# RookieJunChen/FullSubNet-plus

Hardware: AMD Instinct MI355X
Metric: STFT frames/sec (257-bin, 2 s clips), FullSubNet+ forward (higher is better)
Workload: dtype f32

## Files before the change

### fullsubnet_plus_amd/csrc/fsnp_debug_abi.hip

```cpp
#include <algorithm>
#include <string>

#include "fsnp_common.h"
#include "lstm_common.h"
#include "planner.h"
#include "fsnp_handle.h"
#include "weight_layouts.h"
#include "pcm.h"

static double lstm_flops_per_step(const fsnp_handle* h) {
    if (h->sb_tcn) return 8 * (2.0 * h->NIN * h->CH + 2.0 * h->CH * 3 + 2.0 * h->CH * h->NIN) + 2.0 * h->NIN * h->cfg.output_size;
    const double H = h->H, NIN = h->NIN, OUT = h->cfg.output_size, G = h->NG;
    return 2.0 * G * H * (NIN + H) + 2.0 * G * H * (2 * H) + 2.0 * H * OUT;
}
static double tcn_flops_per_frame(const fsnp_handle* h) {
    const double F = h->F, CH = h->CH;
    return h->NB * (2.0 * F * CH + 2.0 * CH * 3 + 2.0 * CH * F) + 2.0 * F * F;
}
static double fb_lstm_flops_per_frame(const fsnp_handle* h) {
    const double F = h->F, CH = h->CH;
    return 2.0 * h->NG * CH * (F + CH) + 2.0 * h->NG * CH * (2 * CH) + 2.0 * CH * F;
}

extern "C" {

int fsnp_read_stage(fsnp_handle* h, const char* name, float* host_out, int64_t numel) {
    if (!h || !name || !host_out) { set_error("fsnp_read_stage: null argument"); return 1; }
    if (!h->have_last) { set_error("fsnp_read_stage: no forward has run"); return 2; }
    const Dims& d = h->last_dims;
    const Workspace& w = h->last_ws;
    const size_t plane = (size_t)d.B * d.Tp * d.FP;
    const std::string n = name;
    const float* src = nullptr;
    bool is_gate = false;
    static const char* tags[3] = {"mag", "real", "imag"};
    for (int b = 0; b < h->NFB; ++b) {
        if (n == std::string("att_") + tags[b]) src = reinterpret_cast<float*>(h->last_base + w.att) + b * plane;
        if (n == std::string("fb_") + tags[b]) src = reinterpret_cast<float*>(h->last_base + w.fb) + b * plane;
        if (h->NFB == 3 && n == std::string("gate_") + tags[b]) { src = reinterpret_cast<float*>(h->last_base + w.gate) + (size_t)b * d.B * d.FP; is_gate = true; }
    }
    if (n == "tcn0_mag") {
        if (!h->debug) { set_error("tcn0_mag needs FSNP_DEBUG_STAGES=1 at fsnp_create time"); return 2; }
        src = reinterpret_cast<float*>(h->last_base + w.dbg_tcn0);
    }
    if (!src) { set_error("unknown stage %s", name); return 2; }
    const int64_t rows = is_gate ? d.B : (int64_t)d.B * d.Tp;
    if (numel != rows * d.F) { set_error("stage %s has %lld elements, caller asked %lld", name, (long long)(rows * d.F), (long long)numel); return 2; }
    FSNP_ON_DEVICE(h);
    FSNP_HIP_CHECK(hipDeviceSynchronize());
    FSNP_HIP_CHECK(hipMemcpy2D(host_out, (size_t)d.F * 4, src, (size_t)d.FP * 4, (size_t)d.F * 4, (size_t)rows, hipMemcpyDeviceToHost));
    return 0;
}

int fsnp_set_timing(fsnp_handle* h, int32_t enable) {
    if (!h) { set_error("null handle"); return 1; }
    h->timing = enable != 0;
    return 0;
}

int fsnp_get_timing(fsnp_handle* h, double ms[4], int64_t count[4], int32_t reset) {
    if (!h || !ms || !count) { set_error("fsnp_get_timing: null argument"); return 1; }
    FSNP_ON_DEVICE(h);
    if (drain_timing(h)) return 1;
    for (int i = 0; i < 4; ++i) { ms[i] = h->acc_ms[i]; count[i] = h->acc_cnt[i]; }
    if (reset) for (int i = 0; i < 4; ++i) { h->acc_ms[i] = 0; h->acc_cnt[i] = 0; }
    return 0;
}

int fsnp_debug_plan_rows(int32_t num_rows, int32_t num_cus, int32_t hidden, int32_t gru, int32_t coop, double composite_gain,
                         int32_t* out, int32_t max_chunks) {
    return fsnp_debug_plan_rows2(num_rows, num_cus, hidden, gru, coop, composite_gain, 1, nullptr, out, max_chunks);
}

static PlannerCtx host_ctx(int32_t num_cus, int32_t hidden, int32_t gru, int32_t coop, double composite_gain, int32_t workgroups_per_cu,
                           const double* costs) {
    PlannerSwitches sw;
    sw.lstm_coop = coop; sw.coop_occ = workgroups_per_cu >= 2 ? 2 : 1;
    PlannerCtx h;
    static_cast<PlannerOptions&>(h) = planner_options(gru ? FSNP_SEQ_GRU : FSNP_SEQ_LSTM, hidden, 34, false, sw);
    h.rowtile_ok = gru != 1;
    h.H = hidden; h.NIN = 34; h.num_cus = num_cus; h.num_cus_real = num_cus; h.gru = gru != 0; h.composite_gain = composite_gain;
    for (int i = 0; i < 4; ++i) h.occ_ksplit[i] = h.coop_occ;
    for (int i = 0; i < 2; ++i) h.occ_coopn[i] = h.coop_occ;
    h.cost = default_costs();
    if (costs) costs_from_array(h.cost, costs);
    if (gru == 2) h.cost.rowtile *= 0.75;
    return h;
}

int fsnp_debug_plan_rows2(int32_t num_rows, int32_t num_cus, int32_t hidden, int32_t gru, int32_t coop, double composite_gain,
                          int32_t workgroups_per_cu, const double* costs, int32_t* out, int32_t max_chunks) {
    if (!out || num_rows <= 0 || num_cus <= 0 || hidden < 128 || hidden % 128 != 0 || max_chunks <= 0) { set_error("fsnp_debug_plan_rows: bad argument"); return -1; }
    const PlannerCtx h = host_ctx(num_cus, hidden, gru, coop, composite_gain, workgroups_per_cu, costs);
    const SbPlan plan = plan_sb(h, num_rows);
    int n = 0;
    for (const SbChunk& c : plan.chunks) {
        if (n >= max_chunks) break;
        int32_t* o = out + 8 * n;
        o[0] = (int)c.kind; o[1] = c.row0; o[2] = c.nrows; o[3] = c.num_tiles; o[4] = c.ex; o[5] = c.kind == SbKind::KSplit || c.kind == SbKind::WaveOwned ? c.units : c.groups;
        o[6] = c.rpg; o[7] = c.slot0;
        ++n;
    }
    return n;
}

int fsnp_debug_coop_side_by_side(const int32_t a_per_xcd[8], int32_t a_own_cu, int32_t a_per_cu, const int32_t b_per_xcd[8],
                                 int32_t b_own_cu, int32_t b_per_cu, int32_t cus_per_xcd) {
    if (!a_per_xcd || !b_per_xcd) { set_error("fsnp_debug_coop_side_by_side: null argument"); return -1; }
    CoopFootprint a{}, b{};
    for (int x = 0; x < kNumXcds; ++x) {
        if (a_per_xcd[x] < 0 || b_per_xcd[x] < 0) { set_error("fsnp_debug_coop_side_by_side: negative workgroup count"); return -1; }
        a.per_xcd[x] = a_per_xcd[x]; b.per_xcd[x] = b_per_xcd[x];
    }
    a.own_cu = a_own_cu != 0; a.per_cu = a_per_cu; b.own_cu = b_own_cu != 0; b.per_cu = b_per_cu;
    return coop_side_by_side(a, b, cus_per_xcd) ? 1 : 0;
}

int fsnp_debug_fullsubnet_pairing(int32_t batch, int32_t num_cus, int32_t fb_workgroups_per_cu, const double* costs, int32_t* out,
                                  int32_t max_records) {
    if (!out || batch <= 0 || num_cus <= 0 || max_records <= 0) { set_error("fsnp_debug_fullsubnet_pairing: bad argument"); return -1; }
    const PlannerCtx c = host_ctx(num_cus, 384, 0, 1, 0.97, 1, costs);
    const int per_cu[3] = {fb_workgroups_per_cu, fb_workgroups_per_cu, fb_workgroups_per_cu};
    return pipeline_pairing(c, true, 257, 512, batch, per_cu, batch <= 4, out, max_records);
}

int fsnp_debug_pipeline_pairing(const fsnp_handle* h, int32_t batch, int32_t* out, int32_t max_records) {
    if (!h || !out || batch <= 0 || max_records <= 0) { set_error("fsnp_debug_pipeline_pairing: bad argument"); return -1; }
    if (!h->committed) { set_error("fsnp_debug_pipeline_pairing: weights not committed (the decision depends on the kernels' occupancy)"); return -1; }
    if (h->model != FSNP_MODEL_FULLSUBNET || h->generic_fb || h->sb_tcn) return 0;
    const bool valu = h->fb_valu && lstm_fbv_available(h->fbw, batch, h->num_cus_real);
    return pipeline_pairing(pctx(h), h->defer_small != 0, h->F, h->CH, batch, h->occ_fb, valu, out, max_records);
}

int fsnp_debug_fullband_launch(const fsnp_handle* h, int32_t batch, int32_t out[4]) {
    if (!h || !out || batch <= 0) { set_error("fsnp_debug_fullband_launch: bad argument"); return 1; }
    if (h->model != FSNP_MODEL_FULLSUBNET) { set_error("fsnp_debug_fullband_launch: FullSubNet+ has no full-band LSTM"); return 2; }
    const FbShape f = fb_shape(h, batch);
    out[0] = (int)f.kernel; out[1] = f.tiles; out[2] = f.rows_per_tile; out[3] = f.units;
    return 0;
}

int fsnp_debug_coop_chain_stats(fsnp_handle* h, int64_t out[2], int32_t reset) {
    if (!h || !out) { set_error("fsnp_debug_coop_chain_stats: null argument"); return 1; }
    take_coop_chain_stats(h, out, reset != 0);
    return 0;
}

int fsnp_get_costs(const fsnp_handle* h, double out[FSNP_NUM_COSTS], int32_t* calibrated, int32_t* occ) {
    if (!h || !out) { set_error("fsnp_get_costs: null argument"); return 1; }
    static_assert(kNumCosts == FSNP_NUM_COSTS, "planner.h and fsnp.h agree on the flat table");
    costs_to_array(h->planner.cost, out);
    if (calibrated) *calibrated = h->planner.cost.calibrated;
    if (occ) *occ = h->planner.coop_occ;
    return 0;
}

int fsnp_measure_costs(fsnp_handle* h, double out[FSNP_NUM_COSTS]) {
    if (!h || !out) { set_error("fsnp_measure_costs: null argument"); return 1; }
    if (!h->committed) { set_error("fsnp_measure_costs: weights not committed"); return 2; }
    if (h->sb_tcn) { set_error("fsnp_measure_costs: the sub-band model of this handle is a TCN (no recurrent kernels)"); return 2; }
    FSNP_ON_DEVICE(h);
    CostTable t = h->planner.cost;
    if (calibrate_costs(h, false, &t)) return 4;
    costs_to_array(t, out);
    return 0;
}

int fsnp_debug_set_costs(fsnp_handle* h, const double* costs, int32_t workgroups_per_cu) {
    if (!h || (workgroups_per_cu != 1 && workgroups_per_cu != 2)) { set_error("fsnp_debug_set_costs: bad argument"); return 1; }
    if (!h->committed) { set_error("fsnp_debug_set_costs: commit the weights first (the kernels' occupancy is checked then)"); return 2; }
    h->planner.cost = initial_costs(h->H, h->gru != 0, h->sb_tcn != 0);
    if (costs) costs_from_array(h->planner.cost, costs);
    h->planner.cost.calibrated = 1;
    h->planner.coop_occ = workgroups_per_cu;
    return 0;
}

int fsnp_describe_plan(const fsnp_handle* h, int32_t batch, int32_t mode, int32_t* out, int32_t max_chunks) {
    if (!h || !out || batch <= 0 || max_chunks <= 0) { set_error("fsnp_describe_plan: bad argument"); return -1; }
    const SbPlan plan = plan_sb(h, batch * rows_per_utt(h, mode));
    int n = 0;
    for (const SbChunk& c : plan.chunks) {
        if (n >= max_chunks) break;
        out[4 * n + 0] = describe_code(c.kind, h->sb_tcn != 0, h->lw.hp_wave && lstm_hpw_available(h->lw));
        out[4 * n + 1] = c.nrows; out[4 * n + 2] = c.num_tiles; out[4 * n + 3] = c.ex;
        ++n;
    }
    return n;
}

int fsnp_describe_plan_ex(const fsnp_handle* h, int32_t batch, int32_t mode, int32_t* out, int32_t max_chunks) {
    if (!h || !out || batch <= 0 || max_chunks <= 0) { set_error("fsnp_describe_plan_ex: bad argument"); return -1; }
    int32_t base[4 * 64];
    const int n = fsnp_describe_plan(h, batch, mode, base, max_chunks < 64 ? max_chunks : 64);
    if (n < 0) return n;
    const SbPlan plan = plan_sb(h, batch * rows_per_utt(h, mode));
    const int first_deferred = plan_first_deferred(h, plan);
    for (int i = 0; i < n; ++i) {
        const SbChunk& c = plan.chunks[i];
        for (int k = 0; k < 4; ++k) out[7 * i + k] = base[4 * i + k];
        int prec = 0;
        if (!h->sb_tcn && !h->gru && c.kind == SbKind::RowTile) prec = h->ih_bf16 == 1 ? 1 : 0;
        if (!h->sb_tcn && !h->gru && c.kind == SbKind::HalfTile && h->ih_bf16 == 1 && h->lw.wpack16_bf) prec = 1;
        out[7 * i + 4] = prec;
        out[7 * i + 5] = h->sb_tcn ? 0 : chunk_workgroups(h, c);
        out[7 * i + 6] = i >= first_deferred ? 1 : 0;
    }
    return n;
}

int fsnp_debug_lstm_profile(fsnp_handle* h, const float* x, float* out, int32_t num_seq, int32_t steps,
                            uint64_t* host_stamps, int64_t num_stamps) {
    if (!h || !x || !out || !host_stamps) { set_error("fsnp_debug_lstm_profile: null argument"); return 1; }
    if (!h->committed) { set_error("fsnp_debug_lstm_profile: weights not committed"); return 2; }
    if (num_stamps != (int64_t)steps * 8) { set_error("fsnp_debug_lstm_profile: need steps*8 stamps"); return 2; }
    if (h->gru || h->sb_tcn || h->H != 384) { set_error("fsnp_debug_lstm_profile: row-tile kernel only (LSTM, hidden 384)"); return 2; }
    FSNP_ON_DEVICE(h);
    const LstmPlan lp = plan_lstm_tiles(num_seq, h->num_cus);
    const int num_slots = lp.num_tiles * lp.rows_per_slot_tile;
    const size_t stamp_off = align_up((size_t)num_slots * sizeof(RowDesc), 256);
    if (ensure_workspace(h, stamp_off + ((size_t)num_stamps + (size_t)lp.num_tiles * 256) * 8, nullptr)) return 4;
    FSNP_HIP_CHECK(hipDeviceSynchronize());
    RowDesc* rows = reinterpret_cast<RowDesc*>(h->ws);
    unsigned long long* dprof = reinterpret_cast<unsigned long long*>(h->ws + stamp_off);
    h->have_last = false;
    launch_build_rows(rows, {num_seq, lp.num_tiles, lp.rows_per_slot_tile, 0}, dense_rows(steps, 2), nullptr);
    LstmArgs a{};
    a.rows = rows; a.dense = x; a.out = out; a.out_stride_o = steps;
    a.num_rows = num_seq; a.num_tiles = lp.num_tiles; a.ex = lp.ex; a.Tp = steps; a.LA = 0; a.F = 1;
    a.act = h->cfg.sb_act; a.prof = dprof;
    launch_lstm(h->lw, a, 0);
    FSNP_HIP_CHECK(hipDeviceSynchronize());
    FSNP_HIP_CHECK(hipMemcpy(host_stamps, dprof, (size_t)num_stamps * 8, hipMemcpyDeviceToHost));
    return 0;
}

int fsnp_debug_pp_profile(fsnp_handle* h, const float* x, float* out, int32_t num_seq, int32_t steps, int32_t tiles_per_group,
                          uint64_t* host_stamps, int64_t num_stamps) {
    if (!h || !x || !out || !host_stamps) { set_error("fsnp_debug_pp_profile: null argument"); return 1; }
    if (!h->committed || (!h->planner.hp_ok && tiles_per_group == 0)) { set_error("fsnp_debug_pp_profile: no half-tile ping-pong kernel for this handle"); return 2; }
    const bool hp = tiles_per_group == 0, cw = tiles_per_group == 32 || tiles_per_group == 64 || tiles_per_group == 96;
    if ((!hp && !cw) || num_stamps != (int64_t)steps * (hp ? 32 : 16)) { set_error("fsnp_debug_pp_profile: tiles_per_group must be 0 (half-tile ping-pong kernel, steps * 32 stamps) or 32 / 64 (wave-owned column split, steps * 16 stamps)"); return 2; }
    if (cw && !h->planner.coopw_ok) { set_error("fsnp_debug_pp_profile: no wave-owned column split for this handle"); return 2; }
    const int tiles = cdiv(num_seq, 32), groups = tiles, S = hp ? h->H / 16 : h->H / tiles_per_group;
    if (num_seq <= 0 || groups * S > h->num_cus_real) { set_error("fsnp_debug_pp_profile: the launch must fit the chip"); return 2; }
    FSNP_ON_DEVICE(h);
    SbPlan plan;
    plan.chunks = {hp ? column_chunk(SbKind::HalfTilePingPong, 0, num_seq, tiles, 16, 0) : column_chunk(SbKind::WaveOwned, 0, num_seq, tiles, tiles_per_group, 0)};
    plan.total_slots = tiles * 32; plan.coop_tiles = tiles;
    const size_t rows_b = align_up((size_t)plan.total_slots * sizeof(RowDesc), 256), hx_b = align_up(lstm_coop_exchange_bytes(h->H, tiles), 256);
    const size_t bar_b = align_up(coop_counter_bytes(tiles), 256), st_b = (size_t)num_stamps * 8;
    if (order_after_last_forward(h, nullptr)) return 4;
    if (ensure_workspace(h, rows_b + hx_b + bar_b + 256 + st_b, nullptr)) return 4;
    FSNP_HIP_CHECK(hipDeviceSynchronize());
    h->have_last = false;
    RowDesc* rows = reinterpret_cast<RowDesc*>(h->ws);
    FSNP_HIP_CHECK(hipMemsetAsync(h->ws + rows_b, 0, hx_b + bar_b + 256 + st_b, nullptr));
    launch_build_rows(plan, rows, dense_rows(steps, h->cfg.output_size), nullptr);
    LstmArgs a{};
    a.rows = rows; a.dense = x; a.dense_stride = h->NIN; a.out = out; a.out_stride_o = steps;
    a.num_rows = num_seq; a.Tp = steps; a.LA = 0; a.FP = 0; a.F = 1; a.NSBN = 0; a.act = h->cfg.sb_act;
    a.prof = reinterpret_cast<unsigned long long*>(h->ws + rows_b + hx_b + bar_b + 256);
    launch_sb_lstm(h, plan, a, reinterpret_cast<float*>(h->ws + rows_b), reinterpret_cast<unsigned*>(h->ws + rows_b + hx_b),
                   reinterpret_cast<unsigned*>(h->ws + rows_b + hx_b + bar_b), nullptr);
    FSNP_HIP_CHECK(hipDeviceSynchronize());
    FSNP_HIP_CHECK(hipMemcpy(host_stamps, a.prof, st_b, hipMemcpyDeviceToHost));
    return fsnp_check_errors(h);
}

int fsnp_debug_launch_clock(fsnp_handle* h, double out[FSNP_LAUNCH_CLOCK_VALUES]) {
    if (!h || !out) { set_error("fsnp_debug_launch_clock: null argument"); return 1; }
    unsigned long long c[8] = {};
    if (!h->d_clk) { set_error("fsnp_debug_launch_clock: no completed launch of the one-tile-per-CU LSTM kernel on this handle"); return 2; }
    FSNP_ON_DEVICE(h);
    FSNP_HIP_CHECK(hipMemcpy(c, h->d_clk, sizeof(c), hipMemcpyDeviceToHost));
    const unsigned long long t0 = c[0], r0 = c[1], t1 = c[2], r1 = c[3];
    if (r0 == 0 || r1 <= r0 || t1 <= t0) { set_error("fsnp_debug_launch_clock: no completed launch of the one-tile-per-CU LSTM kernel on this handle"); return 2; }
    out[0] = (double)(t1 - t0); out[1] = (double)(r1 - r0);
    out[2] = (double)(r1 - r0) * 1e-5;
    out[3] = (double)(t1 - t0) / (double)(r1 - r0) * 100.0;
    out[4] = (double)c[4] * 1e-5;
    out[5] = c[6] == ~0ull ? 0.0 : (double)c[6] * 1e-5;
    out[6] = (double)c[5];
    return 0;
}

int fsnp_debug_verify_sample_stats(const fsnp_handle* h, int64_t out[3]) {
    if (!h || !out) { set_error("fsnp_debug_verify_sample_stats: null argument"); return 1; }
    out[0] = h->vs_runs; out[1] = h->vs_skipped; out[2] = h->vs_calls;
    return 0;
}

int fsnp_debug_corrupt_exchange(fsnp_handle* h, int32_t step) {
    if (!h || step < 0) { set_error("fsnp_debug_corrupt_exchange: step must be >= 0 (0 = off)"); return 1; }
    h->corrupt_exchange = step;
    return 0;
}

int fsnp_debug_inject_error(fsnp_handle* h) {
    if (!h) { set_error("null handle"); return 1; }
    *reinterpret_cast<volatile unsigned*>(h->d_err) |= kErrTimeout;
    return 0;
}

int fsnp_debug_set_chaos(fsnp_handle* h, int32_t seed) {
    if (!h) { set_error("null handle"); return 1; }
    h->coop_chaos = seed;
    return 0;
}

int fsnp_debug_set_gemm_dma(fsnp_handle* h, int32_t mode) {
    if (!h || mode < 0 || mode > 3) { set_error("fsnp_debug_set_gemm_dma: mode must be 0 (general GEMM kernel), 1 (DMA kernels where they apply), 2 (as 1, never the small-batch split-K kernel) or 3 (the 128-row DMA kernel only)"); return 1; }
    h->tw.gemm_dma = mode;
    return 0;
}

int fsnp_debug_set_lstm_coop(fsnp_handle* h, int32_t mode) {
    if (!h || mode < 0 || mode > 4 || mode == 3) { set_error("fsnp_debug_set_lstm_coop: mode must be 0 (off), 1 (auto), 2 (auto, serial K-split schedule, no half-tile ping-pong kernel) or 4 (auto + the half-tile ping-pong kernel even where FSNP_COOP_HP=0)"); return 1; }
    h->planner.lstm_coop = mode != 0;
    h->coop_skew = mode != 2;
    h->planner.coop_hp = mode == 4 ? 1 : mode == 1 ? h->coop_hp_cfg : 0;
    h->fb_valu = mode == 1 || mode == 4;
    h->planner.cost.calibrated = h->calibrate ? 0 : h->planner.cost.calibrated;
    if (!h->planner.cost.calibrated) h->planner.cost = initial_costs(h->H, h->gru != 0, h->sb_tcn != 0);
    return 0;
}

int fsnp_debug_set_lstm_waves(fsnp_handle* h, int32_t waves) {
    if (!h || (waves != 0 && waves != 4 && waves != 12)) { set_error("fsnp_debug_set_lstm_waves: waves must be 0 (auto), 4 or 12"); return 1; }
    h->lstm_waves = waves;
    h->lw.waves = waves;
    return 0;
}

int fsnp_debug_set_num_cus(fsnp_handle* h, int32_t num_cus) {
    if (!h || num_cus <= 0) { set_error("fsnp_debug_set_num_cus: bad argument"); return 1; }
    h->num_cus = num_cus;
    h->tw.num_cus = num_cus;
    return 0;
}

int fsnp_debug_lstm_pack(int32_t hidden, int32_t input_size, int32_t kx, int32_t waves, const float* wih0, const float* whh0,
                         const float* wih1, const float* whh1, float* out, int64_t out_floats) {
    if (!wih0 || !whh0 || !wih1 || !whh1 || !out) { set_error("fsnp_debug_lstm_pack: null argument"); return 1; }
    if (waves <= 0 || hidden % (32 * waves) != 0 || kx % 8 != 0 || input_size > kx) { set_error("fsnp_debug_lstm_pack: bad sizes"); return 2; }
    if (rnn_image_floats(PK_ROWTILE, hidden, input_size, kx, waves) != out_floats) {
        set_error("fsnp_debug_lstm_pack: need %lld floats", (long long)rnn_image_floats(PK_ROWTILE, hidden, input_size, kx, waves));
        return 2;
    }
    pack_rnn_host(PK_ROWTILE, hidden, input_size, kx, waves, wih0, whh0, wih1, whh1, out);
    return 0;
}

int fsnp_debug_lstm_coop_pack(int32_t hidden, int32_t input_size, int32_t kx, int32_t units, const float* wih0, const float* whh0,
                              const float* wih1, const float* whh1, float* out, int64_t out_floats) {
    if (!wih0 || !whh0 || !wih1 || !whh1 || !out) { set_error("fsnp_debug_lstm_coop_pack: null argument"); return 1; }
    if ((units != 8 && units != 16 && units != 32 && units != 64) || hidden % 64 != 0 || kx % 8 != 0 || input_size > kx) {
        set_error("fsnp_debug_lstm_coop_pack: bad sizes");
        return 2;
    }
    if (rnn_image_floats(PK_KSPLIT, hidden, input_size, kx, units) != out_floats) {
        set_error("fsnp_debug_lstm_coop_pack: need %lld floats", (long long)rnn_image_floats(PK_KSPLIT, hidden, input_size, kx, units));
        return 2;
    }
    pack_rnn_host(PK_KSPLIT, hidden, input_size, kx, units, wih0, whh0, wih1, whh1, out);
    return 0;
}

int fsnp_debug_lstm_hpw_pack(int32_t hidden, int32_t input_size, int32_t kx, const float* wih0, const float* whh0, const float* wih1,
                             const float* whh1, float* out, int64_t out_floats) {
    if (!wih0 || !whh0 || !wih1 || !whh1 || !out) { set_error("fsnp_debug_lstm_hpw_pack: null argument"); return 1; }
    if (hidden % 16 != 0 || kx % 4 != 0 || kx > 64 || input_size > kx) { set_error("fsnp_debug_lstm_hpw_pack: bad sizes"); return 2; }
    if (out_floats != rnn_image_floats(PK_HPW, hidden, input_size, kx, 0)) {
        set_error("fsnp_debug_lstm_hpw_pack: need %lld floats", (long long)rnn_image_floats(PK_HPW, hidden, input_size, kx, 0));
        return 2;
    }
    pack_rnn_host(PK_HPW, hidden, input_size, kx, 0, wih0, whh0, wih1, whh1, out);
    return 0;
}

int fsnp_debug_lstm_coopw_pack(int32_t hidden, int32_t input_size, int32_t kx, const float* wih0, const float* whh0, const float* wih1,
                               const float* whh1, float* out, int64_t out_floats) {
    if (!wih0 || !whh0 || !wih1 || !whh1 || !out) { set_error("fsnp_debug_lstm_coopw_pack: null argument"); return 1; }
    if (hidden % 32 != 0 || kx % 8 != 0 || input_size > kx) { set_error("fsnp_debug_lstm_coopw_pack: bad sizes"); return 2; }
    if (rnn_image_floats(PK_COOPW, hidden, input_size, kx, 0) != out_floats) {
        set_error("fsnp_debug_lstm_coopw_pack: need %lld floats", (long long)rnn_image_floats(PK_COOPW, hidden, input_size, kx, 0));
        return 2;
    }
    pack_rnn_host(PK_COOPW, hidden, input_size, kx, 0, wih0, whh0, wih1, whh1, out);
    return 0;
}

int fsnp_debug_lstm_fbv_pack(int32_t hidden, int32_t input_size, const float* wih0, const float* whh0, const float* wih1, const float* whh1,
                             float* out, int64_t out_floats) {
    if (!wih0 || !whh0 || !wih1 || !whh1 || !out) { set_error("fsnp_debug_lstm_fbv_pack: null argument"); return 1; }
    if (hidden != 512 || input_size < 1 || input_size > 288) { set_error("fsnp_debug_lstm_fbv_pack: hidden 512, <= 288 inputs"); return 2; }
    if (rnn_image_floats(PK_FBV, hidden, input_size, 0, 0) != out_floats) {
        set_error("fsnp_debug_lstm_fbv_pack: need %lld floats", (long long)rnn_image_floats(PK_FBV, hidden, input_size, 0, 0));
        return 2;
    }
    pack_rnn_host(PK_FBV, hidden, input_size, 0, 0, wih0, whh0, wih1, whh1, out);
    return 0;
}

double fsnp_lstm_flops(const fsnp_handle* h, int64_t num_seq, int32_t steps) {
    if (!h) return 0;
    return (double)num_seq * steps * lstm_flops_per_step(h);
}

double fsnp_forward_flops(const fsnp_handle* h, int32_t batch, int32_t frames, int32_t mode) {
    if (!h) return 0;
    const double Tp = frames + h->cfg.look_ahead;
    const double full_band = h->model == FSNP_MODEL_FULLSUBNET ? fb_lstm_flops_per_frame(h) : 3.0 * tcn_flops_per_frame(h);
    return batch * Tp * (rows_per_utt(h, mode) * lstm_flops_per_step(h) + full_band);
}

int fsnp_debug_weight_blob(fsnp_handle* h, void* host_dst, int64_t bytes, int64_t* needed) {
    if (!h) { set_error("fsnp_debug_weight_blob: null handle"); return 1; }
    if (!h->committed || !h->d_weights) { set_error("fsnp_debug_weight_blob: weights not committed"); return 2; }
    const int64_t need = (int64_t)(h->blob_floats * sizeof(float));
    if (needed) *needed = need;
    if (!host_dst) return 0;
    if (bytes < need) { set_error("fsnp_debug_weight_blob: need %lld bytes", (long long)need); return 2; }
    FSNP_ON_DEVICE(h);
    FSNP_HIP_CHECK(hipDeviceSynchronize());
    FSNP_HIP_CHECK(hipMemcpy(host_dst, h->d_weights, (size_t)need, hipMemcpyDeviceToHost));
    return 0;
}

const void* fsnp_debug_weight_blob_ptr(const fsnp_handle* h) { return h ? h->d_weights : nullptr; }

int fsnp_debug_commit_stats(const fsnp_handle* h, int64_t out[4]) {
    if (!h || !out) { set_error("fsnp_debug_commit_stats: null argument"); return 1; }
    for (int i = 0; i < 4; ++i) out[i] = h->commit_stats[i];
    return 0;
}

int fsnp_debug_pack_emulate(int32_t kind, const int32_t* sizes, int32_t num_sizes, const float* const* sources, const int64_t* numels,
                            int32_t num_sources, float* out, int64_t out_floats) {
    if (!sizes || !sources || !numels || !out) { set_error("fsnp_debug_pack_emulate: null argument"); return 1; }
    if (kind < 0 || kind >= PK_COUNT || num_sizes < 1 || num_sizes > 5) { set_error("fsnp_debug_pack_emulate: unknown kind / size count"); return 2; }
    int p[5] = {0, 0, 0, 0, 0};
    for (int i = 0; i < num_sizes; ++i) {
        if (sizes[i] < 0) { set_error("fsnp_debug_pack_emulate: negative size"); return 2; }
        p[i] = sizes[i];
    }
    const bool rnn = kind <= PK_SPREAD;
    const int want_sources = rnn ? 8 : kind == PK_FOLDW ? 2 : kind == PK_FOLDC ? 4 : 1;
    bool ok = p[0] > 0 && num_sources == want_sources;
    if (rnn && kind != PK_BIAS) ok = ok && p[1] > 0;
    if (kind <= PK_FBV) ok = ok && p[0] % 8 == 0;
    if (kind == PK_ROWTILE || kind == PK_ROWTILE_BF || kind == PK_GRU) ok = ok && p[3] > 0 && p[0] % (32 * p[3]) == 0 && p[2] % 8 == 0 && p[1] <= p[2];
    if (kind == PK_ROWTILE_BF) ok = ok && p[1] < p[2] && p[0] % 16 == 0;
    if (kind == PK_HALF || kind == PK_HALF_BF) ok = ok && p[0] % 64 == 0 && p[1] <= p[2];
    if (kind == PK_KSPLIT) ok = ok && p[3] >= 8 && p[3] % 8 == 0 && p[0] % p[3] == 0 && p[0] % 16 == 0 && (4 * p[3]) % 32 == 0 && p[2] % 8 == 0 && p[1] <= p[2] && (coop_kgxp(p[2]) + p[0] / 8) % 4 == 0;
    if (kind == PK_COOPN || kind == PK_COOPW) ok = ok && p[0] % 32 == 0 && p[2] % 8 == 0 && p[1] <= p[2];
    if (kind == PK_HP || kind == PK_HPW) ok = ok && p[0] % 16 == 0 && p[1] <= 16 * gx16(p[2]);
    if (kind == PK_FBV) ok = ok && p[0] == 512 && p[1] <= kFbvXP;
    if (kind == PK_SPREAD) ok = ok && p[3] < 4;
    if (kind == PK_PADMAT || kind == PK_FOLDW) ok = ok && p[1] > 0 && p[0] <= p[2] && p[1] <= p[3];
    if (kind == PK_TRANSPOSE) ok = ok && p[1] > 0;
    if (kind == PK_FOLDC) ok = ok && p[1] > 0 && p[0] <= p[2] && p[3] <= 1;
    if (!ok) { set_error("fsnp_debug_pack_emulate: bad sizes / source count for kind %d", kind); return 2; }
    PackJob J = make_job(kind, p[0], p[1], p[2], p[3], p[4]);
    if (J.n != out_floats) { set_error("fsnp_debug_pack_emulate: need %lld floats", (long long)J.n); return 2; }
    std::vector<float> arena;
    for (int i = 0; i < num_sources; ++i) {
        if (numels[i] < 0 || (numels[i] > 0 && !sources[i])) { set_error("fsnp_debug_pack_emulate: source %d is null / negative", i); return 1; }
        J.s[i] = (long long)arena.size();
        arena.insert(arena.end(), sources[i], sources[i] + numels[i]);
    }
    auto inside = [&](int a, long long i) { return a < num_sources && i >= 0 && i < numels[a]; };
    if (kind == PK_FOLDC) {
        if (numels[0] < (int64_t)p[0] * p[1] || numels[1] < p[1] || numels[2] < p[1] || numels[3] < p[0]) {
            set_error("fsnp_debug_pack_emulate: a source of the fold is too small"); return 2;
        }
    } else {
        for (long long u = 0; 4 * u < J.n; ++u) {
            const int nj = pack_unit_bf16(J, u) ? 8 : 4;
            for (int j = 0; j < nj; ++j) {
                long long shift;
                const PackRef r = pack_ref(J, u, j, &shift);
                if (r.a < 0) continue;
                if (!inside(r.a, shift + r.ia) || (r.op != OP_ONE && !inside(r.b, shift + r.ib))) {
                    set_error("fsnp_debug_pack_emulate: kind %d, unit %lld: source offset outside its tensor", kind, u);
                    return 3;
                }
            }
        }
    }
    pack_image_host(J, arena.data(), out, J.n);
    return 0;
}

int fsnp_debug_pcm_convert(fsnp_handle* h, const float* dev_in, int16_t* dev_out, int32_t rows, int32_t n, const int32_t* samples,
                           int32_t out_format, int32_t* dev_clipped, void* stream) {
    if (!h || !dev_in || !dev_out) { set_error("fsnp_debug_pcm_convert: null argument"); return 1; }
    if (rows < 1 || n < 1) { set_error("fsnp_debug_pcm_convert: empty input"); return 2; }
    if (out_format != FSNP_SAMPLE_S16 && out_format != FSNP_SAMPLE_S16_PEAK) {
        set_error("fsnp_debug_pcm_convert: out_format %d is neither FSNP_SAMPLE_S16 nor FSNP_SAMPLE_S16_PEAK", (int)out_format);
        return 2;
    }
    for (int b = 0; samples && b < rows; ++b)
        if (samples[b] < 0 || samples[b] > n) { set_error("fsnp_debug_pcm_convert: row %d: %d samples outside [0, n = %d]", b, (int)samples[b], n); return 2; }
    hipStream_t s = static_cast<hipStream_t>(stream);
    FSNP_ON_DEVICE(h);
    PcmOut out{dev_out, n, 1, kPcmS16, nullptr, nullptr};
    if (dev_clipped) FSNP_HIP_CHECK(hipMemsetAsync(dev_clipped, 0, (size_t)rows * 4, s));
    if (out_format == FSNP_SAMPLE_S16) {
        out.clipped = dev_clipped;
        launch_pcm_convert(dev_in, n, out, rows, n, samples, s);
    } else {
        const size_t stage_b = align_up((size_t)rows * n * 4, 256);
        if (order_after_last_forward(h, s)) return 4;
        if (ensure_io(h, stage_b + (size_t)rows * 4, s)) return 4;
        float* stage = reinterpret_cast<float*>(h->io);
        unsigned* peak = reinterpret_cast<unsigned*>(h->io + stage_b);
        FSNP_HIP_CHECK(hipMemsetAsync(peak, 0, (size_t)rows * 4, s));
        launch_pcm_convert(dev_in, n, PcmOut{stage, n, 1, kPcmPeak, nullptr, peak}, rows, n, samples, s);
        launch_pcm_peak_scale(stage, n, peak, out, rows, n, s);
    }
    FSNP_HIP_CHECK(hipGetLastError());
    return mark_forward_done(h, s);
}

}
```

### fullsubnet_plus_amd/csrc/fsnp_weights.hip

```cpp
#include <algorithm>
#include <cstdlib>
#include <cstring>
#include <string>
#include <vector>

#include "fsnp_handle.h"
#include "weight_layouts.h"
#include "weight_watch.h"

namespace fsnp {

static const int kDilations[8] = {1, 2, 5, 9, 1, 2, 5, 9};
static const char* kAtt[3] = {"channel_attention", "channel_attention_real", "channel_attention_imag"};
static const char* kFb[3] = {"fb_model", "fb_model_real", "fb_model_imag"};
static const char* kConvNames[3] = {"smallConv1d", "middleConv1d", "largeConv1d"};

static void list_specs(fsnp_handle* h) {
    auto add = [&](const std::string& n, int64_t numel) { h->specs.push_back({n, numel}); };
    const int F = h->F, CH = h->CH, H = h->H, Fr = h->Fr;
    const int att = h->cfg.attention;
    const bool fsn = h->model == FSNP_MODEL_FULLSUBNET;
    if (fsn) {
        const std::string f = "fb_model.sequence_model.";
        const int64_t G = h->NG;
        add(f + "weight_ih_l0", G * CH * F);
        add(f + "weight_hh_l0", G * CH * CH);
        add(f + "bias_ih_l0", G * CH);
        add(f + "bias_hh_l0", G * CH);
        add(f + "weight_ih_l1", G * CH * CH);
        add(f + "weight_hh_l1", G * CH * CH);
        add(f + "bias_ih_l1", G * CH);
        add(f + "bias_hh_l1", G * CH);
        add("fb_model.fc_output_layer.weight", (int64_t)F * CH);
        add("fb_model.fc_output_layer.bias", F);
    }
    for (int a = 0; a < 3 && !fsn; ++a) {
        const std::string p = kAtt[a];
        if (att == FSNP_ATT_TSSE) {
            for (int c = 0; c < 3; ++c) {
                add(p + "." + kConvNames[c] + ".0.weight", (int64_t)F * h->cfg.kersize[c]);
                add(p + "." + kConvNames[c] + ".0.bias", F);
            }
            add(p + ".feature_concate_fc.weight", 3);
            add(p + ".feature_concate_fc.bias", 1);
        }
        if (att == FSNP_ATT_ECA) {
            add(p + ".conv.weight", 3);
        } else {
            add(p + ".fc1.weight", (int64_t)Fr * F);
            add(p + ".fc1.bias", Fr);
            add(p + ".fc2.weight", (int64_t)F * Fr);
            add(p + ".fc2.bias", F);
        }
    }
    for (int b = 0; b < 3 && !fsn; ++b) {
        for (int i = 0; i < h->NB; ++i) {
            const std::string p = std::string(kFb[b]) + ".sequence_model." + std::to_string(i);
            add(p + ".conv1x1.weight", (int64_t)CH * F);
            add(p + ".conv1x1.bias", CH);
            add(p + ".prelu1.weight", 1);
            add(p + ".norm1.weight", CH);
            add(p + ".norm1.bias", CH);
            add(p + ".depthwise_conv.weight", (int64_t)CH * 3);
            add(p + ".depthwise_conv.bias", CH);
            add(p + ".prelu2.weight", 1);
            add(p + ".norm2.weight", CH);
            add(p + ".norm2.bias", CH);
            add(p + ".sconv.weight", (int64_t)F * CH);
            add(p + ".sconv.bias", F);
        }
        add(std::string(kFb[b]) + ".fc_output_layer.weight", (int64_t)F * F);
        add(std::string(kFb[b]) + ".fc_output_layer.bias", F);
    }
    if (h->sb_tcn) {
        for (int i = 0; i < 8; ++i) {
            const std::string p = "sb_model.sequence_model." + std::to_string(i);
            add(p + ".conv1x1.weight", (int64_t)CH * h->NIN);
            add(p + ".conv1x1.bias", CH);
            add(p + ".prelu1.weight", 1);
            add(p + ".norm1.weight", CH);
            add(p + ".norm1.bias", CH);
            add(p + ".depthwise_conv.weight", (int64_t)CH * 3);
            add(p + ".depthwise_conv.bias", CH);
            add(p + ".prelu2.weight", 1);
            add(p + ".norm2.weight", CH);
            add(p + ".norm2.bias", CH);
            add(p + ".sconv.weight", (int64_t)h->NIN * CH);
            add(p + ".sconv.bias", h->NIN);
        }
        add("sb_model.fc_output_layer.weight", (int64_t)h->cfg.output_size * h->NIN);
        add("sb_model.fc_output_layer.bias", h->cfg.output_size);
        return;
    }
    const std::string s = "sb_model.sequence_model.";
    const int64_t G = h->NG;
    add(s + "weight_ih_l0", G * H * h->NIN);
    add(s + "weight_hh_l0", G * H * H);
    add(s + "bias_ih_l0", G * H);
    add(s + "bias_hh_l0", G * H);
    add(s + "weight_ih_l1", G * H * H);
    add(s + "weight_hh_l1", G * H * H);
    add(s + "bias_ih_l1", G * H);
    add(s + "bias_hh_l1", G * H);
    add("sb_model.fc_output_layer.weight", (int64_t)h->cfg.output_size * H);
    add("sb_model.fc_output_layer.bias", h->cfg.output_size);
}

void build_specs(fsnp_handle* h) {
    list_specs(h);
    long long at = 0;
    for (size_t i = 0; i < h->specs.size(); ++i) {
        h->spec_off.push_back(at);
        h->spec_index[h->specs[i].name] = (int)i;
        at += h->specs[i].numel;
    }
    h->arena_floats = at;
    h->spec_src.assign(h->specs.size(), 0);
    h->host_arena.assign((size_t)at, 0.0f);
}

__global__ __launch_bounds__(256) void weight_watch_kernel(const WatchSeg* __restrict__ segs, int nseg, unsigned long long* acc,
                                                           int baseline, unsigned* err_host) {
    weight_watch_block(segs, nseg, acc, baseline, err_host, (int)blockIdx.x, (int)gridDim.x);
}
int launch_weight_watch(fsnp_handle* h, hipStream_t s, bool baseline) {
    if (h->watch_nseg <= 0) return 0;
    const int grid = h->watch_nseg < kWatchBlocks ? h->watch_nseg : kWatchBlocks;
    hipLaunchKernelGGL(weight_watch_kernel, dim3(grid), dim3(256), 0, s, static_cast<const WatchSeg*>(h->watch_segs), h->watch_nseg,
                       h->watch_acc, baseline ? 1 : 0, h->d_err);
    FSNP_HIP_CHECK(hipGetLastError());
    return 0;
}
void drop_weight_watch(fsnp_handle* h) {
    if (h->watch_segs) (void)hipFree(h->watch_segs);
    if (h->watch_acc) (void)hipFree(h->watch_acc);
    h->watch_segs = nullptr; h->watch_acc = nullptr; h->watch_nseg = 0;
}

}

extern "C" {

int fsnp_watch_weights(fsnp_handle* h, const void* const* dev_ptrs, const int64_t* numels, int32_t n, int32_t every, void* hip_stream) {
    if (!h || n < 0 || (n > 0 && (!dev_ptrs || !numels)) || every < 1) { set_error("fsnp_watch_weights: bad argument"); return 1; }
    if (!h->committed) { set_error("fsnp_watch_weights: commit the weights first (the baseline fingerprint belongs to the packed set)"); return 2; }
    FSNP_ON_DEVICE(h);
    FSNP_HIP_CHECK(hipDeviceSynchronize());
    drop_weight_watch(h);
    h->watch_every = every; h->watch_calls = 0;
    if (n == 0) return 0;
    std::vector<WatchSeg> segs;
    unsigned long long first = 0;
    constexpr int64_t kSeg = kWatchSeg;
    for (int i = 0; i < n; ++i) {
        if (!dev_ptrs[i] || numels[i] < 0) { set_error("fsnp_watch_weights: tensor %d is null / negative", i); return 1; }
        for (int64_t o = 0; o < numels[i]; o += kSeg) {
            const int64_t c = numels[i] - o < kSeg ? numels[i] - o : kSeg;
            segs.push_back(WatchSeg{static_cast<const unsigned*>(dev_ptrs[i]) + o, (unsigned)c, first + (unsigned long long)o});
        }
        first += (unsigned long long)numels[i];
    }
    if (segs.empty()) return 0;
    FSNP_HIP_CHECK(hipMalloc(&h->watch_segs, segs.size() * sizeof(WatchSeg)));
    FSNP_HIP_CHECK(hipMalloc(reinterpret_cast<void**>(&h->watch_acc), (8 + kWatchBlocks) * 8));
    FSNP_HIP_CHECK(hipMemcpy(h->watch_segs, segs.data(), segs.size() * sizeof(WatchSeg), hipMemcpyHostToDevice));
    FSNP_HIP_CHECK(hipMemsetAsync(h->watch_acc, 0, (8 + kWatchBlocks) * 8, static_cast<hipStream_t>(hip_stream)));
    h->watch_nseg = (int)segs.size();
    if (const int rc = launch_weight_watch(h, static_cast<hipStream_t>(hip_stream), true)) return rc;
    return mark_forward_done(h, static_cast<hipStream_t>(hip_stream));
}

int fsnp_num_weights(const fsnp_handle* h) { return h ? (int)h->specs.size() : 0; }

int fsnp_weight_info(const fsnp_handle* h, int index, const char** name, int64_t* numel) {
    if (!h || index < 0 || index >= (int)h->specs.size()) { set_error("fsnp_weight_info: bad index"); return 1; }
    if (name) *name = h->specs[index].name.c_str();
    if (numel) *numel = h->specs[index].numel;
    return 0;
}

}

namespace fsnp {

int order_after_weight_pack(fsnp_handle* h, hipStream_t s) {
    if (h->packed_valid && h->packed_stream != s) FSNP_HIP_CHECK(hipStreamWaitEvent(s, h->ev_packed, 0));
    return 0;
}

static int find_spec(fsnp_handle* h, const char* name, int64_t numel) {
    const auto it = h->spec_index.find(name);
    if (it == h->spec_index.end()) { set_error("unexpected key in state_dict: %s", name); return -1; }
    const WeightSpec& s = h->specs[it->second];
    if (s.numel != numel) {
        set_error("size mismatch for %s: expected %lld elements, got %lld", name, (long long)s.numel, (long long)numel);
        return -1;
    }
    return it->second;
}

static int download_device_given(fsnp_handle* h, int64_t* bytes) {
    *bytes = 0;
    bool any = false;
    for (unsigned char v : h->spec_src) any = any || v == 2;
    if (!any) return 0;
    FSNP_ON_DEVICE(h);
    FSNP_HIP_CHECK(hipDeviceSynchronize());
    for (size_t i = 0; i < h->specs.size(); ++i) {
        if (h->spec_src[i] != 2) continue;
        const size_t nb = (size_t)h->specs[i].numel * sizeof(float);
        FSNP_HIP_CHECK(hipMemcpy(h->host_arena.data() + h->spec_off[i], h->d_arena + h->spec_off[i], nb, hipMemcpyDeviceToHost));
        h->spec_src[i] = 3;
        *bytes += (int64_t)nb;
    }
    return 0;
}

static int commit_impl(fsnp_handle* h, bool on_device, hipStream_t s) {
    const int F = h->F, CH = h->CH, H = h->H, NB = h->NB, Fr = h->Fr;
    std::vector<PackJob> jobs;
    size_t total = 0;
    auto alloc = [&](size_t n) { const size_t o = total; total = align_up(o + n, 64); return o; };
    auto off = [&](const std::string& n) { return h->spec_off[h->spec_index.at(n)]; };
    auto numel = [&](const std::string& n) { return h->specs[h->spec_index.at(n)].numel; };
    auto emit = [&](PackJob J, size_t o, size_t n) { J.out = (long long)o; J.n = (long long)n; if (n) jobs.push_back(J); };
    auto put = [&](const std::string& n) {
        const int c = (int)numel(n);
        const size_t o = alloc(c);
        PackJob J = make_job(PK_PADMAT, 1, c, 1, c);
        J.s[0] = off(n);
        emit(J, o, c);
        return o;
    };
    auto transposed = [&](const std::string& n, int R, int C) {
        const size_t o = alloc((size_t)R * C);
        PackJob J = make_job(PK_TRANSPOSE, R, C);
        J.s[0] = off(n);
        emit(J, o, (size_t)R * C);
        return o;
    };

    size_t o_conv_w[3][3] = {}, o_conv_b[3][3] = {}, o_cat_w[3] = {}, o_cat_b[3] = {}, o_fc1w[3] = {}, o_fc1b[3] = {},
           o_fc2w[3] = {}, o_fc2b[3] = {};
    const int att = h->cfg.attention;
    const bool fsn = h->model == FSNP_MODEL_FULLSUBNET;
    const int nbr_w = fsn ? 0 : 3;
    for (int a = 0; a < nbr_w; ++a) {
        const std::string p = kAtt[a];
        if (att == FSNP_ATT_TSSE) {
            for (int c = 0; c < 3; ++c) {
                o_conv_w[a][c] = put(p + "." + kConvNames[c] + ".0.weight");
                o_conv_b[a][c] = put(p + "." + kConvNames[c] + ".0.bias");
            }
            o_cat_w[a] = put(p + ".feature_concate_fc.weight");
            o_cat_b[a] = put(p + ".feature_concate_fc.bias");
        }
        if (att == FSNP_ATT_ECA) {
            o_cat_w[a] = put(p + ".conv.weight");
            continue;
        }
        o_fc1w[a] = transposed(p + ".fc1.weight", Fr, F);
        o_fc2w[a] = transposed(p + ".fc2.weight", F, Fr);
        o_fc1b[a] = put(p + ".fc1.bias");
        o_fc2b[a] = put(p + ".fc2.bias");
    }
    struct TcnOff { size_t w1, b1, a1, g1w, g1b, dw, db, a2, g2w, g2b, w2, b2, w2g, c1, c2, wf, bf; int NB, N1P, K1P, N2P, K2P; };
    bool regular = true;
    auto pack_tcn = [&](const std::vector<std::string>& models, int nb, int cin, int fc_out) {
        TcnOff t{};
        const size_t nm = models.size() ? models.size() : 1;
        t.NB = nb; t.N1P = (int)align_up(CH, 384); t.K1P = (int)align_up(cin, 16); t.N2P = (int)align_up(cin, 384); t.K2P = (int)align_up(CH, 16);
        const int nimg = models.empty() ? 0 : (int)(nm * nb), nfc = models.empty() ? 0 : (int)nm;
        auto blk = [&](size_t b, int i, const char* leaf) { return off(models[b] + ".sequence_model." + std::to_string(i) + leaf); };
        auto fc = [&](size_t b, const char* leaf) { return off(models[b] + ".fc_output_layer" + leaf); };
        auto image = [&](PackJob J, size_t size, std::initializer_list<const char*> leaves, bool per_block) {
            const size_t o = alloc(size);
            J.nsub = per_block ? nimg : nfc;
            J.nb = per_block ? nb : 1;
            if (J.nsub > 0) {
                int k = 0;
                for (const char* leaf : leaves) {
                    J.s[k] = per_block ? blk(0, 0, leaf) : fc(0, leaf);
                    if (per_block) {
                        J.stride_in = nb > 1 ? blk(0, 1, leaf) - J.s[k] : 0;
                        J.stride_out = nm > 1 ? blk(1, 0, leaf) - J.s[k] : 0;
                        for (size_t b = 0; b < nm; ++b)
                            for (int i = 0; i < nb; ++i) regular = regular && blk(b, i, leaf) == J.s[k] + (long long)b * J.stride_out + i * J.stride_in;
                    } else {
                        J.stride_out = nm > 1 ? fc(1, leaf) - J.s[k] : 0;
                        for (size_t b = 0; b < nm; ++b) regular = regular && fc(b, leaf) == J.s[k] + (long long)b * J.stride_out;
                    }
                    ++k;
                }
            }
            emit(J, o, size);
            return o;
        };
        auto vec = [&](int len, int padded) { return make_job(PK_PADMAT, 1, len, 1, padded); };
        t.w1 = image(make_job(PK_PADMAT, CH, cin, t.N1P, t.K1P), nm * nb * t.N1P * t.K1P, {".conv1x1.weight"}, true);
        t.b1 = image(vec(CH, t.N1P), nm * nb * t.N1P, {".conv1x1.bias"}, true);
        t.a1 = image(vec(1, 1), nm * nb + 1, {".prelu1.weight"}, true);
        t.g1w = image(vec(CH, CH), nm * nb * CH, {".norm1.weight"}, true);
        t.g1b = image(vec(CH, CH), nm * nb * CH, {".norm1.bias"}, true);
        t.dw = image(make_job(PK_TRANSPOSE, CH, 3), nm * nb * 3 * CH, {".depthwise_conv.weight"}, true);
        t.db = image(vec(CH, CH), nm * nb * CH, {".depthwise_conv.bias"}, true);
        t.a2 = image(vec(1, 1), nm * nb + 1, {".prelu2.weight"}, true);
        t.g2w = image(vec(CH, CH), nm * nb * CH, {".norm2.weight"}, true);
        t.g2b = image(vec(CH, CH), nm * nb * CH, {".norm2.bias"}, true);
        t.w2 = image(make_job(PK_PADMAT, cin, CH, t.N2P, t.K2P), nm * nb * t.N2P * t.K2P, {".sconv.weight"}, true);
        t.b2 = image(vec(cin, t.N2P), nm * nb * t.N2P, {".sconv.bias"}, true);
        t.w2g = image(make_job(PK_FOLDW, cin, CH, t.N2P, t.K2P), nm * nb * t.N2P * t.K2P, {".sconv.weight", ".norm2.weight"}, true);
        t.c1 = image(make_job(PK_FOLDC, cin, CH, t.N2P, 0), nm * nb * t.N2P, {".sconv.weight", ".norm2.weight", ".norm2.bias", ".sconv.bias"}, true);
        t.c2 = image(make_job(PK_FOLDC, cin, CH, t.N2P, 1), nm * nb * t.N2P, {".sconv.weight", ".norm2.weight", ".norm2.bias", ".sconv.bias"}, true);
        t.wf = image(make_job(PK_PADMAT, fc_out, cin, t.N2P, t.K1P), nm * t.N2P * t.K1P, {".weight"}, false);
        t.bf = image(vec(fc_out, t.N2P), nm * t.N2P, {".bias"}, false);
        return t;
    };
    auto bind_tcn = [&](TcnWeights& t, const TcnOff& o, const float* d) {
        t.w1 = d + o.w1; t.b1 = d + o.b1; t.a1 = d + o.a1; t.g1w = d + o.g1w; t.g1b = d + o.g1b;
        t.dw = d + o.dw; t.db = d + o.db; t.a2 = d + o.a2; t.g2w = d + o.g2w; t.g2b = d + o.g2b;
        t.w2 = d + o.w2; t.b2 = d + o.b2; t.wf = d + o.wf; t.bf = d + o.bf;
        t.w2g = d + o.w2g; t.c1 = d + o.c1; t.c2 = d + o.c2;
        t.num_cus = h->num_cus; t.NB = o.NB; t.N1P = o.N1P; t.K1P = o.K1P; t.N2P = o.N2P; t.K2P = o.K2P;
        for (int i = 0; i < o.NB; ++i) t.dilation[i] = kDilations[i];
        const char* de = getenv("FSNP_GEMM_DMA");
        t.gemm_dma = de && de[0] == '0' ? 0 : 1;
    };
    std::vector<std::string> fb_models;
    for (int b = 0; b < nbr_w; ++b) fb_models.push_back(kFb[b]);
    const TcnOff fb_off = pack_tcn(fb_models, NB, F, F);
    const TcnOff sb_off = h->sb_tcn ? pack_tcn({"sb_model"}, 8, h->NIN, h->cfg.output_size) : TcnOff{};
    if (!regular) { set_error("fsnp_commit_weights: the TCN blocks are not evenly spaced in the parameter list"); return 3; }
    auto rnn = [&](int kind, const std::string& pre, int Hh, int nin, int kx, int P) {
        PackJob J = make_job(kind, Hh, nin, kx, P, h->gru);
        static const char* leaves[8] = {"weight_ih_l0", "weight_hh_l0", "weight_ih_l1", "weight_hh_l1", "bias_ih_l0", "bias_hh_l0", "bias_ih_l1", "bias_hh_l1"};
        for (int i = 0; i < 8; ++i) J.s[i] = off(pre + leaves[i]);
        const size_t o = alloc((size_t)J.n);
        emit(J, o, (size_t)J.n);
        return o;
    };
    const std::string sbp = "sb_model.sequence_model.";
    auto sb = [&](int kind, int P = 0) { return rnn(kind, sbp, H, h->NIN, h->KX, P); };
    const bool tuned = !h->sb_tcn && !h->generic_sb;
    size_t o_wgen = 0;
    if (h->generic_sb) o_wgen = sb(PK_GENERIC);
    size_t o_wpack = 0, o_wpack12 = 0, o_wpack_bf[2] = {0, 0};
    if (!h->gru && tuned && (H == 384 || H == 256)) {
        o_wpack = sb(PK_ROWTILE, 4);
        if (H == 384) o_wpack12 = sb(PK_ROWTILE, 12);
        for (int i = 0; i < 2 && h->KX == 40 && H == 384 && h->NIN < h->KX; ++i) o_wpack_bf[i] = sb(PK_ROWTILE_BF, i == 0 ? 4 : 12);
    }
    size_t o_wpack16 = 0, o_wpack16_bf = 0;
    bool have16_bf = false;
    if (h->planner.lstm16_ok) {
        o_wpack16 = sb(PK_HALF);
        if (h->KX == 40 && H == 384) {
            o_wpack16_bf = sb(PK_HALF_BF);
            have16_bf = true;
        }
    }
    size_t o_wpack_gru = 0;
    if (h->gru && tuned && H == 384) o_wpack_gru = sb(PK_GRU, 4);
    size_t o_wpack_coop[4] = {0, 0, 0, 0};
    for (int ui = 0; ui < 4 && tuned; ++ui) o_wpack_coop[ui] = sb(PK_KSPLIT, 8 << ui);
    size_t o_wpack_hp = 0, o_wpack_hpw = 0;
    if (h->planner.hp_ok) {
        o_wpack_hp = sb(PK_HP);
        o_wpack_hpw = sb(PK_HPW);
    }
    size_t o_wpack_coopw = 0;
    if (h->planner.coopw_ok) o_wpack_coopw = sb(PK_COOPW);
    const size_t o_wpack_coopn = tuned ? sb(PK_COOPN) : alloc(0);
    constexpr int KXF = 264;
    size_t o_fbpack[3] = {0, 0, 0}, o_fbbias = 0, o_fsn_wf = 0, o_fsn_bf = 0, o_fbgen = 0, o_fbv = 0;
    bool have_fbv = false;
    const int fsn_kp = (int)align_up(CH, 16), fsn_np = (int)align_up(F, 384);
    if (fsn) {
        const std::string fbp = "fb_model.sequence_model.";
        if (h->generic_fb || !h->gru) o_fbgen = rnn(PK_GENERIC, fbp, CH, F, 0, 0);
        for (int ui = 0; ui < 3 && !h->generic_fb; ++ui) o_fbpack[ui] = rnn(PK_KSPLIT, fbp, CH, F, KXF, 8 << ui);
        if (!h->generic_fb && !h->gru && CH == 512 && F <= 288) {
            o_fbv = rnn(PK_FBV, fbp, CH, F, 0, 0);
            have_fbv = true;
        }
        o_fbbias = rnn(PK_BIAS, fbp, CH, F, 0, 0);
        o_fsn_wf = alloc((size_t)fsn_np * fsn_kp);
        PackJob J = make_job(PK_PADMAT, F, CH, fsn_np, fsn_kp);
        J.s[0] = off("fb_model.fc_output_layer.weight");
        emit(J, o_fsn_wf, (size_t)fsn_np * fsn_kp);
        o_fsn_bf = alloc(fsn_np);
        PackJob Jb = make_job(PK_PADMAT, 1, F, 1, fsn_np);
        Jb.s[0] = off("fb_model.fc_output_layer.bias");
        emit(Jb, o_fsn_bf, fsn_np);
    }
    const size_t o_lbias = h->sb_tcn ? alloc(0) : sb(PK_BIAS);
    const size_t o_wfc = h->sb_tcn ? 0 : put("sb_model.fc_output_layer.weight");
    const size_t o_bfc = h->sb_tcn ? 0 : put("sb_model.fc_output_layer.bias");
    const size_t o_refl = alloc(F), o_reflfb = alloc(F);
    const size_t refl_floats = total - o_refl;
    if (h->refl_host.size() != refl_floats) {
        h->refl_host.assign(refl_floats, 0.0f);
        for (int f = 0; f < F; ++f) {
            for (int j = 0; j < h->NSB; ++j) h->refl_host[reflect_index(f - h->cfg.sb_num_neighbors + j, F)] += 1.0f;
            for (int j = 0; j < 2 * h->cfg.fb_num_neighbors + 1; ++j) h->refl_host[o_reflfb - o_refl + reflect_index(f - h->cfg.fb_num_neighbors + j, F)] += 1.0f;
        }
    }

    FSNP_ON_DEVICE(h);
    int64_t stats[4] = {on_device ? 1 : 0, 0, 0, 0};
    if (!on_device) {
        std::vector<float> blob(total, 0.0f);
        for (const PackJob& J : jobs) pack_image_host(J, h->host_arena.data(), blob.data() + J.out, (long long)align_up((size_t)J.n, 64));
        std::copy(h->refl_host.begin(), h->refl_host.end(), blob.begin() + o_refl);
        if (h->d_weights) { FSNP_HIP_CHECK(hipDeviceSynchronize()); FSNP_HIP_CHECK(hipFree(h->d_weights)); h->d_weights = nullptr; }
        FSNP_HIP_CHECK(hipMalloc(reinterpret_cast<void**>(&h->d_weights), blob.size() * sizeof(float)));
        FSNP_HIP_CHECK(hipMemcpy(h->d_weights, blob.data(), blob.size() * sizeof(float), hipMemcpyHostToDevice));
        h->blob_floats = total;
        h->packed_valid = false;
        stats[1] = (int64_t)(blob.size() * sizeof(float));
    } else {
        if (order_after_last_forward(h, s)) return 4;
        if (h->pipeline && fsnp_flush(h, s)) return 4;
        if (h->arena_valid && h->arena_stream != s) FSNP_HIP_CHECK(hipStreamWaitEvent(s, h->ev_arena, 0));
        if (h->d_weights && h->blob_floats != total) { FSNP_HIP_CHECK(hipDeviceSynchronize()); FSNP_HIP_CHECK(hipFree(h->d_weights)); h->d_weights = nullptr; }
        if (h->d_weights) FSNP_HIP_CHECK(hipDeviceSynchronize());
        else FSNP_HIP_CHECK(hipMalloc(reinterpret_cast<void**>(&h->d_weights), total * sizeof(float)));
        h->blob_floats = total;
        h->committed = false;
        for (const PackJob& J : jobs) {
            if (const int rc = launch_pack_image(J, h->d_arena, h->arena_floats, h->d_weights, (long long)align_up((size_t)J.n, 64), s)) return rc;
            ++stats[3];
        }
        FSNP_HIP_CHECK(hipMemcpyAsync(h->d_weights + o_refl, h->refl_host.data(), refl_floats * sizeof(float), hipMemcpyHostToDevice, s));
        stats[1] = (int64_t)(refl_floats * sizeof(float));
        if (!h->ev_packed) FSNP_HIP_CHECK(hipEventCreateWithFlags(&h->ev_packed, hipEventDisableTiming));
        FSNP_HIP_CHECK(hipEventRecord(h->ev_packed, s));
        h->packed_stream = s; h->packed_valid = true;
        if (mark_forward_done(h, s)) return 4;
    }
    for (int i = 0; i < 4; ++i) if (i != 2) h->commit_stats[i] = stats[i];
    const float* d = h->d_weights;
    for (int a = 0; a < 3; ++a) {
        for (int c = 0; c < 3; ++c) { h->fw.conv_w[a][c] = d + o_conv_w[a][c]; h->fw.conv_b[a][c] = d + o_conv_b[a][c]; }
        h->fw.cat_w[a] = d + o_cat_w[a]; h->fw.cat_b[a] = d + o_cat_b[a];
        h->fw.fc1_wT[a] = d + o_fc1w[a]; h->fw.fc1_b[a] = d + o_fc1b[a];
        h->fw.fc2_wT[a] = d + o_fc2w[a]; h->fw.fc2_b[a] = d + o_fc2b[a];
    }
    for (int c = 0; c < 3; ++c) h->fw.ksize[c] = h->cfg.kersize[c];
    h->fw.attention = h->cfg.attention;
    h->fw.subband_num = h->cfg.subband_num > 0 ? h->cfg.subband_num : 1;
    bind_tcn(h->tw, fb_off, d);
    h->lw.wpack = d + o_wpack; h->lw.wpack12 = d + o_wpack12; for (int ui = 0; ui < 4; ++ui) h->lw.wpack_coop[ui] = d + o_wpack_coop[ui];
    h->lw.wpack_coopn = d + o_wpack_coopn;
    h->lw.wpack_hp = d + o_wpack_hp;
    h->lw.wpack_hpw = h->planner.hp_ok ? d + o_wpack_hpw : nullptr;
    h->lw.hp_wave = h->hp_wave;
    h->lw.wpack_coopw = h->planner.coopw_ok ? d + o_wpack_coopw : nullptr;
    h->lw.wpack_gru = d + o_wpack_gru;
    h->lw.wpack16 = d + o_wpack16;
    h->lw.wpack16_bf = have16_bf ? d + o_wpack16_bf : nullptr;
    h->lw.wpack_bf[0] = d + o_wpack_bf[0]; h->lw.wpack_bf[1] = d + o_wpack_bf[1]; h->lw.ih_bf16 = h->ih_bf16; h->lw.waves = h->lstm_waves; h->lw.bias = d + o_lbias; h->lw.wfc = d + o_wfc; h->lw.bfc = d + o_bfc;
    h->lw.H = H; h->lw.NIN = h->NIN; h->lw.KX = h->KX; h->lw.OUT = h->cfg.output_size; h->lw.gru = h->gru;
    h->lw.wgen = d + o_wgen;
    if (h->sb_tcn) bind_tcn(h->sbt, sb_off, d);
    if (fsn) {
        h->fbw = LstmWeights{};
        for (int ui = 0; ui < 3; ++ui) h->fbw.wpack_coop[ui] = d + o_fbpack[ui];
        h->fbw.bias = d + o_fbbias;
        h->fbw.H = CH; h->fbw.NIN = F; h->fbw.KX = KXF; h->fbw.OUT = 0; h->fbw.gru = h->gru;
        h->fbw.wgen = d + o_fbgen;
        h->fbw.wpack_fbv = have_fbv ? d + o_fbv : nullptr;
        h->fsn_wf = d + o_fsn_wf; h->fsn_bf = d + o_fsn_bf; h->fsn_kp = fsn_kp;
    }
    h->d_refl_w = d + o_refl;
    h->d_refl_wfb = d + o_reflfb;
    if (tuned) {
        for (int ui = 0; ui < 4; ++ui) h->planner.occ_ksplit[ui] = std::max(1, lstm_coop_occupancy(h->lw, 8 << ui));
        for (int rpg = 1; rpg <= 2; ++rpg) h->planner.occ_coopn[rpg - 1] = std::max(1, lstm_coopn_occupancy(h->lw, rpg));
    }
    for (int ui = 0; ui < 3 && fsn && !h->generic_fb; ++ui) h->occ_fb[ui] = lstm_coop_seq_occupancy(h->fbw, 8 << ui);
    if (h->generic_sb && lstm_generic_check(h->H, h->NIN, false)) return 2;
    if (h->generic_fb && lstm_generic_check(h->CH, h->F, true)) return 2;
    h->committed = true;
    return 0;
}

static int missing_key(const fsnp_handle* h) {
    for (size_t i = 0; i < h->specs.size(); ++i)
        if (!h->spec_src[i]) { set_error("missing key in state_dict: %s", h->specs[i].name.c_str()); return 2; }
    return 0;
}

static int commit_host(fsnp_handle* h) {
    int64_t down = 0;
    if (const int rc = download_device_given(h, &down)) return rc;
    h->commit_stats[2] = down;
    return commit_impl(h, false, nullptr);
}

}

extern "C" {

int fsnp_set_weight(fsnp_handle* h, const char* name, const float* host_data, int64_t numel) {
    if (!h || !name || !host_data) { set_error("fsnp_set_weight: null argument"); return 1; }
    const int i = find_spec(h, name, numel);
    if (i < 0) return 2;
    std::copy(host_data, host_data + numel, h->host_arena.begin() + h->spec_off[i]);
    h->spec_src[i] = 1;
    h->committed = false;
    h->watch_nseg = 0;
    return 0;
}

int fsnp_set_weight_device(fsnp_handle* h, const char* name, const float* dev_data, int64_t numel, void* hip_stream) {
    if (!h || !name || !dev_data) { set_error("fsnp_set_weight_device: null argument"); return 1; }
    const int i = find_spec(h, name, numel);
    if (i < 0) return 2;
    FSNP_ON_DEVICE(h);
    hipStream_t s = static_cast<hipStream_t>(hip_stream);
    if (!h->d_arena) FSNP_HIP_CHECK(hipMalloc(reinterpret_cast<void**>(&h->d_arena), (size_t)std::max<long long>(h->arena_floats, 1) * sizeof(float)));
    if (!h->ev_arena) FSNP_HIP_CHECK(hipEventCreateWithFlags(&h->ev_arena, hipEventDisableTiming));
    if (h->arena_valid && h->arena_stream != s) FSNP_HIP_CHECK(hipStreamWaitEvent(s, h->ev_arena, 0));
    if (const int rc = order_after_weight_pack(h, s)) return rc;
    FSNP_HIP_CHECK(hipMemcpyAsync(h->d_arena + h->spec_off[i], dev_data, (size_t)numel * sizeof(float), hipMemcpyDeviceToDevice, s));
    FSNP_HIP_CHECK(hipEventRecord(h->ev_arena, s));
    h->arena_stream = s; h->arena_valid = true;
    h->spec_src[i] = 2;
    h->committed = false;
    h->watch_nseg = 0;
    return 0;
}

int fsnp_commit_weights(fsnp_handle* h) {
    if (!h) { set_error("null handle"); return 1; }
    if (const int rc = missing_key(h)) return rc;
    return commit_host(h);
}

int fsnp_commit_weights_on(fsnp_handle* h, void* hip_stream) {
    if (!h) { set_error("null handle"); return 1; }
    if (const int rc = missing_key(h)) return rc;
    bool all_device = true;
    for (unsigned char v : h->spec_src) all_device = all_device && v >= 2;
    if (!all_device) return commit_host(h);
    h->commit_stats[2] = 0;
    return commit_impl(h, true, static_cast<hipStream_t>(hip_stream));
}

}
```

### fullsubnet_plus_amd/csrc/lstm.hip

```cpp
#include <cstring>

#include "fsnp_common.h"
#include "lstm_common.h"

namespace fsnp {

template <int EX>
__host__ __device__ __forceinline__ int e_frag_index(int e, int k) {
    return ((((k >> 3) * 2) + (k & 1)) * EX + e) * 4 + ((k >> 1) & 3);
}

struct WStream {
    __amdgpu_buffer_rsrc_t rsrc;
    int voff;
};
template <int NT>
__device__ __forceinline__ float4 wload(const WStream& ws, int g, int n) {
    const auto v = __builtin_amdgcn_raw_buffer_load_b128(ws.rsrc, ws.voff, (g * NT + n) * 1024, 0);
    return __builtin_bit_cast(float4, v);
}

template <int NT, int EX>
__device__ __forceinline__ void mfma_groups(f32x16 (&acc)[NT], float (&accx)[EX > 0 ? EX : 1][NT], float4 (&b)[NT],
                                            const float4* __restrict__ A, const float4* __restrict__ AE, int ngroups,
                                            const WStream& ws, int& gnext, int groups_total) {
    float4 a = A[0];
    float4 ae[EX > 0 ? EX : 1];
#pragma unroll
    for (int e = 0; e < EX; ++e) ae[e] = AE[e];
    for (int g = 0; g < ngroups; ++g) {
        const int gn = (g + 1 < ngroups ? g + 1 : g);
        const float4 an = A[gn * 64];
        float4 aen[EX > 0 ? EX : 1];
#pragma unroll
        for (int e = 0; e < EX; ++e) aen[e] = AE[gn * 2 * EX + e];
        if constexpr (EX == 0) {
#pragma unroll
            for (int n = 0; n < NT; ++n) {
                acc[n] = __builtin_amdgcn_mfma_f32_32x32x2f32(a.x, b[n].x, acc[n], 0, 0, 0);
                acc[n] = __builtin_amdgcn_mfma_f32_32x32x2f32(a.y, b[n].y, acc[n], 0, 0, 0);
                acc[n] = __builtin_amdgcn_mfma_f32_32x32x2f32(a.z, b[n].z, acc[n], 0, 0, 0);
                acc[n] = __builtin_amdgcn_mfma_f32_32x32x2f32(a.w, b[n].w, acc[n], 0, 0, 0);
                b[n] = wload<NT>(ws, gnext, n);
                __builtin_amdgcn_sched_barrier(0);
            }
        } else {
            constexpr int HALF = NT / 2;
#pragma unroll
            for (int hb = 0; hb < NT; hb += HALF) {
#pragma unroll
                for (int n = hb; n < hb + HALF; ++n) {
                    acc[n] = __builtin_amdgcn_mfma_f32_32x32x2f32(a.x, b[n].x, acc[n], 0, 0, 0);
                    acc[n] = __builtin_amdgcn_mfma_f32_32x32x2f32(a.y, b[n].y, acc[n], 0, 0, 0);
                    acc[n] = __builtin_amdgcn_mfma_f32_32x32x2f32(a.z, b[n].z, acc[n], 0, 0, 0);
                    acc[n] = __builtin_amdgcn_mfma_f32_32x32x2f32(a.w, b[n].w, acc[n], 0, 0, 0);
                }
                __builtin_amdgcn_sched_barrier(0);
#pragma unroll
                for (int n = hb; n < hb + HALF; ++n)
#pragma unroll
                    for (int e = 0; e < EX; ++e) {
                        float v = accx[e][n];
                        v = fmaf(ae[e].x, b[n].x, v);
                        v = fmaf(ae[e].y, b[n].y, v);
                        v = fmaf(ae[e].z, b[n].z, v);
                        accx[e][n] = fmaf(ae[e].w, b[n].w, v);
                    }
                __builtin_amdgcn_sched_barrier(0);
#pragma unroll
                for (int n = hb; n < hb + HALF; ++n) b[n] = wload<NT>(ws, gnext, n);
                __builtin_amdgcn_sched_barrier(0);
            }
        }
        gnext = (gnext + 1 == groups_total) ? 0 : gnext + 1;
        a = an;
#pragma unroll
        for (int e = 0; e < EX; ++e) ae[e] = aen[e];
    }
}

__device__ __forceinline__ unsigned short bf16_bits(float v) {
    const unsigned u = __float_as_uint(v);
    return (unsigned short)((u + 0x7FFFu + ((u >> 16) & 1u)) >> 16);
}
__host__ __device__ __forceinline__ int a_frag_index_bf16(int row, int k) {
    return (((k >> 4) * 64) + (((k >> 3) & 1) * 32) + row) * 8 + (k & 7);
}

template <int ST, int UW, int HBLO = 0>
__device__ __forceinline__ void lstm_cell(f32x16 (&acc)[4 * ST], f32x2 (&c)[ST][8], float* __restrict__ Hs, int wave,
                                          int lane, unsigned short* __restrict__ Hb = nullptr) {
#pragma unroll
    for (int s = 0; s < ST; ++s) {
        const int k = wave * UW + s * 32 + (lane & 31);
        const int kbase = (((k >> 3) * 64) + ((k & 1) * 32)) * 4 + ((k >> 1) & 3);
#pragma unroll
        for (int r = 0; r < 16; r += 2) {
            auto rd = [](float v) {
                if constexpr (ST > 1) { float o; asm("v_accvgpr_read_b32 %0, %1" : "=v"(o) : "a"(v)); return o; }
                else return v;
            };
            const f32x2 h = lstm_cell_pair(f32x2{rd(acc[s][r]), rd(acc[s][r + 1])}, f32x2{rd(acc[ST + s][r]), rd(acc[ST + s][r + 1])},
                                           f32x2{rd(acc[2 * ST + s][r]), rd(acc[2 * ST + s][r + 1])},
                                           f32x2{rd(acc[3 * ST + s][r]), rd(acc[3 * ST + s][r + 1])}, c[s][r >> 1]);
            const int row = (r & 3) + 8 * (r >> 2) + 4 * (lane >> 5);
            Hs[kbase + row * 4] = h.x;
            Hs[kbase + (row + 1) * 4] = h.y;
            if (Hb) {
                const unsigned short hx = bf16_bits(h.x), hy = bf16_bits(h.y);
                Hb[a_frag_index_bf16(row, k)] = hx; Hb[a_frag_index_bf16(row + 1, k)] = hy;
                if constexpr (HBLO > 0) {
                    Hb[HBLO + a_frag_index_bf16(row, k)] = bf16_bits(h.x - __uint_as_float((unsigned)hx << 16));
                    Hb[HBLO + a_frag_index_bf16(row + 1, k)] = bf16_bits(h.y - __uint_as_float((unsigned)hy << 16));
                }
            }
        }
    }
}

using bf16x8 = __attribute__((ext_vector_type(8))) __bf16;
template <int NT, int EX, int ALO>
__device__ __forceinline__ void mfma_groups_bf16(f32x16 (&acc)[NT], float (&accx)[EX > 0 ? EX : 1][NT], float4 (&b)[NT],
                                                 const float4* __restrict__ A, const float4* __restrict__ AE, int nsteps,
                                                 const WStream& ws, int& gnext, int groups_total, int lane) {
    float4 a = A[0], al = A[ALO];
    for (int g = 0; g < nsteps; ++g) {
        const float4 an = A[(g + 1 < nsteps ? g + 1 : g) * 64], aln = A[ALO + (g + 1 < nsteps ? g + 1 : g) * 64];
        float4 he[EX > 0 ? EX : 1][2];
        if constexpr (EX > 0) {
            const int kg = 2 * g + (lane >> 5);
#pragma unroll
            for (int e = 0; e < EX; ++e) { he[e][0] = AE[(kg * 2 + 0) * EX + e]; he[e][1] = AE[(kg * 2 + 1) * EX + e]; }
        }
#pragma unroll
        for (int n = 0; n < NT; ++n) {
            if constexpr (EX > 0) {
                const unsigned w0 = __float_as_uint(b[n].x), w1 = __float_as_uint(b[n].y), w2 = __float_as_uint(b[n].z),
                               w3 = __float_as_uint(b[n].w);
#pragma unroll
                for (int e = 0; e < EX; ++e) {
                    float v = accx[e][n];
                    v = fmaf(he[e][0].x, __uint_as_float(w0 << 16), v);
                    v = fmaf(he[e][1].x, __uint_as_float(w0 & 0xFFFF0000u), v);
                    v = fmaf(he[e][0].y, __uint_as_float(w1 << 16), v);
                    v = fmaf(he[e][1].y, __uint_as_float(w1 & 0xFFFF0000u), v);
                    v = fmaf(he[e][0].z, __uint_as_float(w2 << 16), v);
                    v = fmaf(he[e][1].z, __uint_as_float(w2 & 0xFFFF0000u), v);
                    v = fmaf(he[e][0].w, __uint_as_float(w3 << 16), v);
                    accx[e][n] = fmaf(he[e][1].w, __uint_as_float(w3 & 0xFFFF0000u), v);
                }
            }
            acc[n] = __builtin_amdgcn_mfma_f32_32x32x16_bf16(__builtin_bit_cast(bf16x8, a), __builtin_bit_cast(bf16x8, b[n]),
                                                             acc[n], 0, 0, 0);
            if constexpr (ALO > 0)
                acc[n] = __builtin_amdgcn_mfma_f32_32x32x16_bf16(__builtin_bit_cast(bf16x8, al), __builtin_bit_cast(bf16x8, b[n]),
                                                                 acc[n], 0, 0, 0);
            b[n] = wload<NT>(ws, gnext, n);
            __builtin_amdgcn_sched_barrier(0);
        }
        gnext = (gnext + 1 == groups_total) ? 0 : gnext + 1;
        a = an; al = aln;
    }
}

template <int ST, int UW, int EX, int NT>
__device__ __forceinline__ void lstm_cell_extra(float (&accx)[EX > 0 ? EX : 1][NT], float (&cx)[EX > 0 ? EX : 1][ST],
                                                const float* __restrict__ bias, float* __restrict__ He, int wave,
                                                int lane) {
#pragma unroll
    for (int e = 0; e < EX; ++e)
#pragma unroll
        for (int s = 0; s < ST; ++s) {
            float g4[4];
#pragma unroll
            for (int q = 0; q < 4; ++q) {
                const float v = accx[e][q * ST + s];
                g4[q] = v + __shfl_xor(v, 32) + (bias ? bias[(q * ST + s) * 32] : 0.0f);
            }
            const float cn = fast_sigmoid(g4[1]) * cx[e][s] + fast_sigmoid(g4[0]) * fast_tanh(g4[2]);
            cx[e][s] = cn;
            const float h = fast_sigmoid(g4[3]) * fast_tanh(cn);
            if (lane < 32) He[e_frag_index<EX>(e, wave * UW + s * 32 + lane)] = h;
        }
}

template <int HID, int KX, int OUT, int EX, bool PROF, int NW, bool BF>
__global__ __launch_bounds__(64 * NW) __attribute__((amdgpu_waves_per_eu(NW / 4, NW / 4)))
void lstm2_fc_kernel(LstmWeights w, LstmArgs a) {
    static_assert(OUT == 2, "FC lane mapping assumes output_size == 2");
    static_assert(EX >= 0 && EX <= 4, "at most 4 VALU rows per tile (one FC wave per extra row)");
    static_assert(NW % 4 == 0 && NW >= 4, "whole waves per SIMD");
    constexpr int NTHR = 64 * NW;
    constexpr int UW = HID / NW, ST = UW / 32, NT = 4 * ST;
    static_assert(UW % 32 == 0 && UW * NW == HID, "hidden/NW must be a multiple of 32");
    constexpr int KGX = KX / 8, KGH = HID / 8, KG0 = KGX + KGH;
    constexpr int KSB = HID / 16;
    constexpr int KG1 = BF ? KGH + KSB : 2 * KGH, KGT = KG0 + KG1;
    static_assert(KGH % 4 == 0, "FC k-split");
    static_assert(!BF || HID % 16 == 0, "bf16 k-steps");
    constexpr int RT = 32 + EX;
    constexpr int EXA = EX > 0 ? EX : 1;

    extern __shared__ __attribute__((aligned(16))) unsigned char smem_raw[];
    float4* Xs = reinterpret_cast<float4*>(smem_raw);
    float4* H0s = Xs + KGX * 64;
    float4* H1s = H0s + KGH * 64;
    float4* XEs = H1s + KGH * 64;
    float4* HE0s = XEs + KGX * 2 * EX;
    float4* HE1s = HE0s + KGH * 2 * EX;
    float4* Wfc4 = HE1s + KGH * 2 * EX;
    RowDesc* rows_s = reinterpret_cast<RowDesc*>(Wfc4 + OUT * KGH * 2);
    constexpr int BL = BF ? 1 : 2;
    constexpr bool HILO = BF && EX == 0;
    float* Bs = reinterpret_cast<float*>(rows_s + RT);
    float4* H0b = reinterpret_cast<float4*>(Bs + BL * NW * NT * 32);

    const int tid = threadIdx.x;
    const int lane = tid & 63;
    const int wave = __builtin_amdgcn_readfirstlane(tid >> 6);
    const int slot0 = blockIdx.x * RT;
    const int Tp = a.Tp;

    __shared__ unsigned long long clk_s[2];
    if (a.clk != nullptr && tid == 0) {
        clk_s[1] = __builtin_amdgcn_s_memrealtime();
        clk_s[0] = __builtin_amdgcn_s_memtime();
        if (blockIdx.x == 0) { a.clk[0] = clk_s[0]; a.clk[1] = clk_s[1]; a.clk[4] = 0ull; a.clk[5] = 0ull; a.clk[6] = ~0ull; }
    }

    for (int i = tid; i < (KGX + 2 * KGH) * (64 + 2 * EX); i += NTHR) Xs[i] = make_float4(0.f, 0.f, 0.f, 0.f);
    for (int i = tid; i < OUT * KGH * 2; i += NTHR) {
        const int o = i / (KGH * 2), kg = (i >> 1) % KGH, kh = i & 1;
        const float* wr = w.wfc + (size_t)o * HID + kg * 8 + kh;
        Wfc4[i] = make_float4(wr[0], wr[2], wr[4], wr[6]);
    }
    if (tid < RT) rows_s[tid] = a.rows[slot0 + tid];
    for (int i = tid; i < BL * NW * NT * 32; i += NTHR) {
        const int col = i & 31, n = (i >> 5) % NT, wv = (i / (32 * NT)) % NW, layer = BF ? 1 : i / (32 * NT * NW);
        Bs[i] = w.bias[layer * 4 * HID + (n / ST) * HID + wv * UW + (n % ST) * 32 + col];
    }
    __syncthreads();
    if constexpr (BF) {
        if (tid < 32) reinterpret_cast<float*>(Xs)[a_frag_index(tid, w.NIN)] = 1.0f;
        if (EX > 0 && tid < EX) reinterpret_cast<float*>(XEs)[e_frag_index<EXA>(tid, w.NIN)] = 1.0f;
    }

    const bool dense = a.dense != nullptr;
    const float* __restrict__ gbase = dense ? a.dense : a.att_mag;
    const int gstep = dense ? w.NIN : a.FP;
    auto plan = [&](const RowDesc& rd, int j) -> int {
        if (!rd.valid || j >= w.NIN) return -1;
        if (dense) return rd.b * Tp * w.NIN + j;
        return sb_feature_offset(j, rd.f, rd.b * Tp * a.FP, a.F, a.NSBN, a.NFBN, a.fb_rel, a.fb_branch_stride);
    };
    auto row_md = [&](const RowDesc& rd, int slot, NormMD& md, const NormMD*& md_row) {
        md.m = 0.0f; md.d = 1.0f; md_row = nullptr;
        if (dense || !rd.valid) return;
        if (a.md_row != nullptr) md_row = a.md_row + (size_t)slot * Tp;
        else md = a.md_utt[rd.b];
    };
    constexpr int JSTEP = NTHR / 32, NG = (KX + JSTEP - 1) / JSTEP;
    const int grow = tid & 31;
    int goff[NG], xdst[NG];
    NormMD md; const NormMD* md_row;
    {
        const RowDesc rd = rows_s[grow];
#pragma unroll
        for (int i = 0; i < NG; ++i) {
            const int j = (tid >> 5) + JSTEP * i;
            goff[i] = (j < KX && !(BF && j == w.NIN)) ? plan(rd, j) : -2;
            xdst[i] = a_frag_index(grow, j < KX ? j : 0);
        }
        row_md(rd, slot0 + grow, md, md_row);
    }
    int goffx = -1, xdstx = 0;
    NormMD mdx = {0.0f, 1.0f}; const NormMD* mdx_row = nullptr;
    bool havex = EX > 0 && tid < EX * KX;
    if (BF && havex && tid % KX == w.NIN) havex = false;
    if (havex) {
        const int e = tid / KX, j = tid % KX;
        const RowDesc rd = rows_s[32 + e];
        goffx = plan(rd, j);
        xdstx = e_frag_index<EXA>(e, j);
        row_md(rd, slot0 + 32 + e, mdx, mdx_row);
    }

    float* Xf = reinterpret_cast<float*>(Xs);
    float* XEf = reinterpret_cast<float*>(XEs);
    {
        const NormMD m0 = md_row ? md_row[0] : md;
#pragma unroll
        for (int i = 0; i < NG; ++i)
            if (goff[i] != -2) Xf[xdst[i]] = goff[i] >= 0 ? (gbase[goff[i]] - m0.m) / m0.d : 0.0f;
        if (havex) {
            const NormMD mx = mdx_row ? mdx_row[0] : mdx;
            XEf[xdstx] = goffx >= 0 ? (gbase[goffx] - mx.m) / mx.d : 0.0f;
        }
    }

    const float* __restrict__ bias_l0 = BF ? nullptr : Bs + ((0 * NW + wave) * NT) * 32 + (lane & 31);
    const float* __restrict__ bias_l1 = Bs + (((BL - 1) * NW + wave) * NT) * 32 + (lane & 31);
    f32x2 c0[ST][8], c1[ST][8];
    float cx0[EXA][ST], cx1[EXA][ST];
#pragma unroll
    for (int s = 0; s < ST; ++s) {
#pragma unroll
        for (int r = 0; r < 8; ++r) { c0[s][r] = f32x2{0.0f, 0.0f}; c1[s][r] = f32x2{0.0f, 0.0f}; }
#pragma unroll
        for (int e = 0; e < EXA; ++e) { cx0[e][s] = 0.0f; cx1[e][s] = 0.0f; }
    }

    WStream ws;
    ws.rsrc = __builtin_amdgcn_make_buffer_rsrc(const_cast<float*>(w.wpack) + (size_t)wave * KGT * NT * 256, 0,
                                                KGT * NT * 1024, 0x00020000);
    ws.voff = lane * 16;
    float4 breg[NT];
#pragma unroll
    for (int n = 0; n < NT; ++n) breg[n] = wload<NT>(ws, 0, n);
    int gnext = 1;
    auto run_groups = [&](f32x16 (&acc_)[NT], float (&accx_)[EXA][NT], const float4* A_, const float4* AE_, int ng) {
        mfma_groups<NT, EX>(acc_, accx_, breg, A_, AE_, ng, ws, gnext, KGT);
    };

    const int fc_row = (wave & 3) * 8 + (lane & 7);
    const int fc_o = (lane >> 3) & 1;
    const int fc_kp = lane >> 4;
    const RowDesc fc_rd = rows_s[fc_row];
    const RowDesc fcx_rd = (EX > 0 && wave < EX) ? rows_s[32 + (wave < EX ? wave : 0)] : RowDesc{0, 0, 0, 0};

    auto fc_store = [&](int t_of_h) {
      if (wave < 4) {
        constexpr int KGP = KGH / 4;
        float sum = 0.0f;
#pragma unroll 4
        for (int kk = 0; kk < KGP; ++kk) {
            const int kg = fc_kp * KGP + kk;
#pragma unroll
            for (int kh = 0; kh < 2; ++kh) {
                const float4 h4 = H1s[kg * 64 + kh * 32 + fc_row];
                const float4 w4 = Wfc4[(fc_o * KGH + kg) * 2 + kh];
                sum += h4.x * w4.x + h4.y * w4.y + h4.z * w4.z + h4.w * w4.w;
            }
        }
        sum += __shfl_xor(sum, 16);
        sum += __shfl_xor(sum, 32);
        if (fc_kp == 0 && fc_rd.valid && t_of_h >= a.LA)
            a.out[(size_t)fc_rd.out_off + (size_t)fc_o * a.out_stride_o + (t_of_h - a.LA)] = apply_act(sum + w.bfc[fc_o], a.act);
      }
        if (EX > 0 && wave < EX) {
            const int o = lane >> 5;
            const float* he = reinterpret_cast<const float*>(HE1s);
            float sx = 0.0f;
#pragma unroll 4
            for (int i = 0; i < HID / 32; ++i) {
                const int k = (lane & 31) + 32 * i;
                sx += he[e_frag_index<EXA>(wave, k)] * w.wfc[o * HID + k];
            }
#pragma unroll
            for (int m = 16; m > 0; m >>= 1) sx += __shfl_xor(sx, m);
            if ((lane & 31) == 0 && fcx_rd.valid && t_of_h >= a.LA)
                a.out[(size_t)fcx_rd.out_off + (size_t)o * a.out_stride_o + (t_of_h - a.LA)] = apply_act(sx + w.bfc[o], a.act);
        }
    };

    const float4* AEx = XEs + (lane >> 5) * EX;
    const float4* AEh0 = HE0s + (lane >> 5) * EX;
    const float4* AEh1 = HE1s + (lane >> 5) * EX;

    __syncthreads();

    unsigned long long* prof = nullptr;
    int prof_stride = 0;
    if constexpr (PROF) {
        const bool rec = blockIdx.x == 0 && tid == 0;
        prof = a.prof + (rec ? 0 : (size_t)Tp * 8 + (size_t)blockIdx.x * 256 + tid);
        prof_stride = rec ? 8 : 0;
    }
#define FSNP_STAMP(i) do { if constexpr (PROF) prof[t * prof_stride + (prof_stride ? (i) : 0)] = __builtin_amdgcn_s_memtime(); } while (0)

    for (int t = 0; t < Tp; ++t) {
        FSNP_STAMP(0);
        float xr[NG], xrx = 0.0f;
        NormMD mdn = md, mdxn = mdx;
        const bool have_next = (t + 1 < Tp);
        if (have_next) {
            if (md_row) mdn = md_row[t + 1];
#pragma unroll
            for (int i = 0; i < NG; ++i) xr[i] = goff[i] >= 0 ? gbase[goff[i] + (t + 1) * gstep] : 0.0f;
            if (havex) {
                if (mdx_row) mdxn = mdx_row[t + 1];
                xrx = goffx >= 0 ? gbase[goffx + (t + 1) * gstep] : 0.0f;
            }
        }

        f32x16 acc[NT];
        float accx[EXA][NT];
#pragma unroll
        for (int n = 0; n < NT; ++n) {
#pragma unroll
            for (int r = 0; r < 16; ++r) acc[n][r] = BF ? 0.0f : bias_l0[n * 32];
#pragma unroll
            for (int e = 0; e < EXA; ++e) accx[e][n] = 0.0f;
        }
        run_groups(acc, accx, Xs + lane, AEx, KG0);
        FSNP_STAMP(1);
        __syncthreads();
        FSNP_STAMP(2);
        lstm_cell<ST, UW, HILO ? KSB * 64 * 8 : 0>(acc, c0, reinterpret_cast<float*>(H0s), wave, lane, BF ? reinterpret_cast<unsigned short*>(H0b) : nullptr);
        if (EX > 0) lstm_cell_extra<ST, UW, EX, NT>(accx, cx0, bias_l0, reinterpret_cast<float*>(HE0s), wave, lane);
        if (have_next) {
#pragma unroll
            for (int i = 0; i < NG; ++i)
                if (goff[i] != -2) Xf[xdst[i]] = goff[i] >= 0 ? (xr[i] - mdn.m) / mdn.d : 0.0f;
            if (havex) XEf[xdstx] = goffx >= 0 ? (xrx - mdxn.m) / mdxn.d : 0.0f;
        }
        if (t > 0) fc_store(t - 1);
        FSNP_STAMP(3);
        __syncthreads();
        FSNP_STAMP(4);
#pragma unroll
        for (int n = 0; n < NT; ++n) {
#pragma unroll
            for (int r = 0; r < 16; ++r) acc[n][r] = bias_l1[n * 32];
#pragma unroll
            for (int e = 0; e < EXA; ++e) accx[e][n] = 0.0f;
        }
        run_groups(acc, accx, H1s + lane, AEh1, KGH);
        if constexpr (BF) mfma_groups_bf16<NT, EX, HILO ? KSB * 64 : 0>(acc, accx, breg, H0b + lane, HE0s, KSB, ws, gnext, KGT, lane);
        else run_groups(acc, accx, H0s + lane, AEh0, KGH);
        FSNP_STAMP(5);
        __syncthreads();
        FSNP_STAMP(6);
        lstm_cell<ST, UW>(acc, c1, reinterpret_cast<float*>(H1s), wave, lane);
        if (EX > 0) lstm_cell_extra<ST, UW, EX, NT>(accx, cx1, bias_l1, reinterpret_cast<float*>(HE1s), wave, lane);
        FSNP_STAMP(7);
    }
#undef FSNP_STAMP
    __syncthreads();
    fc_store(Tp - 1);
    if (a.clk != nullptr && tid == 0) {
        const unsigned long long m1 = __builtin_amdgcn_s_memtime(), r1 = __builtin_amdgcn_s_memrealtime();
        if (blockIdx.x == 0) { a.clk[2] = m1; a.clk[3] = r1; }
        atomicMax(a.clk + 4, r1 - clk_s[1]);
        atomicMax(a.clk + 5, m1 - clk_s[0]);
        atomicMin(a.clk + 6, r1 - clk_s[1]);
    }
}





template <int EX, int NW, bool BF, int KX, int HID = 384>
static void launch_lstm_ex(const LstmWeights& w, const LstmArgs& a, hipStream_t s) {
    constexpr int OUT = 2;
    constexpr int KGX = KX / 8, KGH = HID / 8, NT = 4 * (HID / NW / 32);
    const size_t smem = (size_t)(KGX + 2 * KGH) * (64 + 2 * EX) * 16 + (size_t)OUT * KGH * 2 * 16 +
                        (32 + EX) * sizeof(RowDesc) + (size_t)(BF ? 1 : 2) * NW * NT * 32 * 4 + (BF ? (size_t)(EX == 0 ? 2 : 1) * (HID / 16) * 64 * 16 : 0);
    LstmWeights wv = w;
    wv.wpack = BF ? (NW == 12 ? w.wpack_bf[1] : w.wpack_bf[0]) : (NW == 12 ? w.wpack12 : w.wpack);
    if constexpr (KX == 40 && HID == 384) {
        if (a.prof != nullptr) {
            auto kern = lstm2_fc_kernel<HID, KX, OUT, EX, true, NW, BF>;
            (void)hipFuncSetAttribute(reinterpret_cast<const void*>(kern), hipFuncAttributeMaxDynamicSharedMemorySize, (int)smem);
            hipLaunchKernelGGL(kern, dim3(a.num_tiles), dim3(64 * NW), smem, s, wv, a);
            return;
        }
    }
    auto kern = lstm2_fc_kernel<HID, KX, OUT, EX, false, NW, BF>;
    static PerDeviceOnce attr_once;
    attr_once.run([&] { (void)hipFuncSetAttribute(reinterpret_cast<const void*>(kern), hipFuncAttributeMaxDynamicSharedMemorySize, (int)smem); });
    hipLaunchKernelGGL(kern, dim3(a.num_tiles), dim3(64 * NW), smem, s, wv, a);
}

template <int NW, bool BF, int KX>
static void launch_lstm_nw(const LstmWeights& w, const LstmArgs& a, hipStream_t s) {
    switch (a.ex) {
        case 0: launch_lstm_ex<0, NW, BF, KX>(w, a, s); break;
        case 1: launch_lstm_ex<1, NW, BF, KX>(w, a, s); break;
        case 2: launch_lstm_ex<2, NW, BF, KX>(w, a, s); break;
        default: launch_lstm_ex<4, NW, BF, KX>(w, a, s); break;
    }
}

void launch_lstm(const LstmWeights& w, const LstmArgs& a, hipStream_t s) {
    if (a.num_tiles <= 0) return;
    const int waves = w.waves != 0 ? w.waves : (a.ex > 0 ? 12 : 4);
    if (w.H == 256) {
        if (w.KX == 64) launch_lstm_ex<0, 4, false, 64, 256>(w, a, s);
        else launch_lstm_ex<0, 4, false, 40, 256>(w, a, s);
        return;
    }
    if (w.KX == 64) {
        if (waves == 12) launch_lstm_nw<12, false, 64>(w, a, s);
        else launch_lstm_nw<4, false, 64>(w, a, s);
    } else if (w.ih_bf16) {
        if (waves == 12) launch_lstm_nw<12, true, 40>(w, a, s);
        else launch_lstm_nw<4, true, 40>(w, a, s);
    } else {
        if (waves == 12) launch_lstm_nw<12, false, 40>(w, a, s);
        else launch_lstm_nw<4, false, 40>(w, a, s);
    }
}

template <int ST, int UW, int HID, bool LOAD>
__device__ __forceinline__ void stream_state_io(f32x2 (&c0)[ST][8], f32x2 (&c1)[ST][8], float* __restrict__ H0, float* __restrict__ H1,
                                                const RowDesc* __restrict__ rows_s, float* __restrict__ state, long slot_stride, int done,
                                                int wave, int lane) {
#pragma unroll
    for (int r = 0; r < 16; ++r) {
        const int row = (r & 3) + 8 * (r >> 2) + 4 * (lane >> 5);
        const RowDesc rd = rows_s[row];
        const bool on = LOAD ? rd.valid > 0 : rd.valid == done;
        float* __restrict__ p = state + (size_t)rd.b * slot_stride + (size_t)rd.f * 4 * HID;
#pragma unroll
        for (int s = 0; s < ST; ++s) {
            const int k = wave * UW + s * 32 + (lane & 31);
            const int hi = (((k >> 3) * 64) + ((k & 1) * 32)) * 4 + ((k >> 1) & 3) + row * 4;
            if constexpr (LOAD) {
                H0[hi] = on ? p[k] : 0.0f;
                c0[s][r >> 1][r & 1] = on ? p[HID + k] : 0.0f;
                H1[hi] = on ? p[2 * HID + k] : 0.0f;
                c1[s][r >> 1][r & 1] = on ? p[3 * HID + k] : 0.0f;
            } else if (on) {
                p[k] = H0[hi];
                p[HID + k] = c0[s][r >> 1][r & 1];
                p[2 * HID + k] = H1[hi];
                p[3 * HID + k] = c1[s][r >> 1][r & 1];
            }
        }
    }
}

template <int HID, int KX>
__global__ __launch_bounds__(256) __attribute__((amdgpu_waves_per_eu(1, 1)))
void lstm2_fc_stream_kernel(LstmWeights w, LstmArgs a) {
    constexpr int NW = 4, NTHR = 256, OUT = 2;
    constexpr int UW = HID / NW, ST = UW / 32, NT = 4 * ST;
    constexpr int KGX = KX / 8, KGH = HID / 8, KG0 = KGX + KGH, KGT = KG0 + 2 * KGH;
    static_assert(UW % 32 == 0 && KGH % 4 == 0, "hidden/4 must be a multiple of 32");

    extern __shared__ __attribute__((aligned(16))) unsigned char smem_raw[];
    float4* Xs = reinterpret_cast<float4*>(smem_raw);
    float4* H0s = Xs + KGX * 64;
    float4* H1s = H0s + KGH * 64;
    float4* Wfc4 = H1s + KGH * 64;
    RowDesc* rows_s = reinterpret_cast<RowDesc*>(Wfc4 + OUT * KGH * 2);
    float* Bs = reinterpret_cast<float*>(rows_s + 32);

    const int tid = threadIdx.x;
    const int lane = tid & 63;
    const int wave = __builtin_amdgcn_readfirstlane(tid >> 6);
    const int slot0 = blockIdx.x * 32;
    const int Tp = a.Tp;

    for (int i = tid; i < (KGX + 2 * KGH) * 64; i += NTHR) Xs[i] = make_float4(0.f, 0.f, 0.f, 0.f);
    for (int i = tid; i < OUT * KGH * 2; i += NTHR) {
        const int o = i / (KGH * 2), kg = (i >> 1) % KGH, kh = i & 1;
        const float* wr = w.wfc + (size_t)o * HID + kg * 8 + kh;
        Wfc4[i] = make_float4(wr[0], wr[2], wr[4], wr[6]);
    }
    if (tid < 32) rows_s[tid] = a.rows[slot0 + tid];
    for (int i = tid; i < 2 * NW * NT * 32; i += NTHR) {
        const int col = i & 31, n = (i >> 5) % NT, wv = (i / (32 * NT)) % NW, layer = i / (32 * NT * NW);
        Bs[i] = w.bias[layer * 4 * HID + (n / ST) * HID + wv * UW + (n % ST) * 32 + col];
    }
    __syncthreads();

    int nsteps = 0, cmin = 1 << 30;
    for (int r = 0; r < 32; ++r) {
        const int v = rows_s[r].valid;
        nsteps = v > nsteps ? v : nsteps;
        if (v > 0) cmin = v < cmin ? v : cmin;
    }
    nsteps = __builtin_amdgcn_readfirstlane(nsteps);
    const bool mixed = __builtin_amdgcn_readfirstlane(cmin < nsteps ? 1 : 0) != 0;
    if (nsteps <= 0) return;

    constexpr int JSTEP = NTHR / 32, NG = (KX + JSTEP - 1) / JSTEP;
    const int grow = tid & 31;
    int goff[NG], xdst[NG];
    const float* __restrict__ gbase = a.att_mag;
    const int gstep = a.FP;
    const NormMD* md_row;
    {
        const RowDesc rd = rows_s[grow];
#pragma unroll
        for (int i = 0; i < NG; ++i) {
            const int j = (tid >> 5) + JSTEP * i;
            goff[i] = j >= KX ? -2 : (rd.valid > 0 && j < w.NIN)
                          ? sb_feature_offset(j, rd.f, rd.b * Tp * a.FP, a.F, a.NSBN, a.NFBN, a.fb_rel, a.fb_branch_stride) : -1;
            xdst[i] = a_frag_index(grow, j < KX ? j : 0);
        }
        md_row = a.md_row + (size_t)(slot0 + grow) * Tp;
    }
    float* Xf = reinterpret_cast<float*>(Xs);
    {
        const NormMD m0 = rows_s[grow].valid > 0 ? md_row[0] : NormMD{0.0f, 1.0f};
#pragma unroll
        for (int i = 0; i < NG; ++i)
            if (goff[i] != -2) Xf[xdst[i]] = goff[i] >= 0 ? (gbase[goff[i]] - m0.m) / m0.d : 0.0f;
    }

    const float* __restrict__ bias_l0 = Bs + ((0 * NW + wave) * NT) * 32 + (lane & 31);
    const float* __restrict__ bias_l1 = Bs + ((1 * NW + wave) * NT) * 32 + (lane & 31);
    f32x2 c0[ST][8], c1[ST][8];
    stream_state_io<ST, UW, HID, true>(c0, c1, reinterpret_cast<float*>(H0s), reinterpret_cast<float*>(H1s), rows_s, a.st_sb, a.st_stride, 0,
                                       wave, lane);

    WStream ws;
    ws.rsrc = __builtin_amdgcn_make_buffer_rsrc(const_cast<float*>(w.wpack) + (size_t)wave * KGT * NT * 256, 0, KGT * NT * 1024, 0x00020000);
    ws.voff = lane * 16;
    float4 breg[NT];
#pragma unroll
    for (int n = 0; n < NT; ++n) breg[n] = wload<NT>(ws, 0, n);
    int gnext = 1;
    float accx[1][NT];
    auto run_groups = [&](f32x16 (&acc_)[NT], const float4* A_, int ng) {
        mfma_groups<NT, 0>(acc_, accx, breg, A_, A_, ng, ws, gnext, KGT);
    };

    const int fc_row = (wave & 3) * 8 + (lane & 7);
    const int fc_o = (lane >> 3) & 1;
    const int fc_kp = lane >> 4;
    const RowDesc fc_rd = rows_s[fc_row];
    auto fc_store = [&](int t_of_h) {
        constexpr int KGP = KGH / 4;
        float sum = 0.0f;
#pragma unroll 4
        for (int kk = 0; kk < KGP; ++kk) {
            const int kg = fc_kp * KGP + kk;
#pragma unroll
            for (int kh = 0; kh < 2; ++kh) {
                const float4 h4 = H1s[kg * 64 + kh * 32 + fc_row];
                const float4 w4 = Wfc4[(fc_o * KGH + kg) * 2 + kh];
                sum += h4.x * w4.x + h4.y * w4.y + h4.z * w4.z + h4.w * w4.w;
            }
        }
        sum += __shfl_xor(sum, 16);
        sum += __shfl_xor(sum, 32);
        if (fc_kp == 0 && t_of_h < fc_rd.valid)
            a.out[(size_t)fc_rd.out_off + (size_t)fc_o * a.out_stride_o + t_of_h] = apply_act(sum + w.bfc[fc_o], a.act);
    };

    __syncthreads();

    for (int t = 0; t < nsteps; ++t) {
        float xr[NG];
        NormMD mdn = {0.0f, 1.0f};
        const bool have_next = (t + 1 < nsteps);
        if (have_next) {
            if (rows_s[grow].valid > 0) mdn = md_row[t + 1];
#pragma unroll
            for (int i = 0; i < NG; ++i) xr[i] = goff[i] >= 0 ? gbase[goff[i] + (t + 1) * gstep] : 0.0f;
        }

        f32x16 acc[NT];
#pragma unroll
        for (int n = 0; n < NT; ++n)
#pragma unroll
            for (int r = 0; r < 16; ++r) acc[n][r] = bias_l0[n * 32];
        run_groups(acc, Xs + lane, KG0);
        __syncthreads();
        lstm_cell<ST, UW>(acc, c0, reinterpret_cast<float*>(H0s), wave, lane);
        if (have_next) {
#pragma unroll
            for (int i = 0; i < NG; ++i)
                if (goff[i] != -2) Xf[xdst[i]] = goff[i] >= 0 ? (xr[i] - mdn.m) / mdn.d : 0.0f;
        }
        if (t > 0) fc_store(t - 1);
        __syncthreads();
#pragma unroll
        for (int n = 0; n < NT; ++n)
#pragma unroll
            for (int r = 0; r < 16; ++r) acc[n][r] = bias_l1[n * 32];
        run_groups(acc, H1s + lane, KGH);
        run_groups(acc, H0s + lane, KGH);
        __syncthreads();
        lstm_cell<ST, UW>(acc, c1, reinterpret_cast<float*>(H1s), wave, lane);
        if (t + 1 == nsteps || mixed)
            stream_state_io<ST, UW, HID, false>(c0, c1, reinterpret_cast<float*>(H0s), reinterpret_cast<float*>(H1s), rows_s, a.st_sb,
                                                a.st_stride, t + 1, wave, lane);
    }
    __syncthreads();
    fc_store(nsteps - 1);
}

template <int HID, int KX>
static void launch_lstm_stream_one(const LstmWeights& w, const LstmArgs& a, hipStream_t s) {
    constexpr int KGX = KX / 8, KGH = HID / 8, NT = 4 * (HID / 4 / 32);
    const size_t smem = (size_t)(KGX + 2 * KGH) * 64 * 16 + (size_t)2 * KGH * 2 * 16 + 32 * sizeof(RowDesc) + (size_t)2 * 4 * NT * 32 * 4;
    auto kern = lstm2_fc_stream_kernel<HID, KX>;
    static PerDeviceOnce attr_once;
    attr_once.run([&] { (void)hipFuncSetAttribute(reinterpret_cast<const void*>(kern), hipFuncAttributeMaxDynamicSharedMemorySize, (int)smem); });
    hipLaunchKernelGGL(kern, dim3(a.num_tiles), dim3(256), smem, s, w, a);
}

bool lstm_stream_available(const LstmWeights& w) {
    return !w.gru && w.OUT == 2 && (w.H == 384 || w.H == 256) && (w.KX == 40 || w.KX == 64) && w.wpack != nullptr;
}

void launch_lstm_stream(const LstmWeights& w, const LstmArgs& a, hipStream_t s) {
    if (a.num_tiles <= 0) return;
    if (w.H == 256) { if (w.KX == 64) launch_lstm_stream_one<256, 64>(w, a, s); else launch_lstm_stream_one<256, 40>(w, a, s); }
    else if (w.KX == 64) launch_lstm_stream_one<384, 64>(w, a, s);
    else launch_lstm_stream_one<384, 40>(w, a, s);
}

LstmPlan plan_lstm_tiles(int num_rows, int num_cus) {
    LstmPlan p{};
    if (num_rows <= 32 * num_cus) {
        p.ex = 0; p.num_tiles = cdiv(num_rows, 32);
    } else {
        const int cand[4] = {0, 1, 2, 4};
        int best_rounds = 1 << 30;
        for (int i = 0; i < 4; ++i) {
            const int rounds = cdiv(cdiv(num_rows, 32 + cand[i]), num_cus);
            if (rounds < best_rounds) { best_rounds = rounds; p.ex = cand[i]; }
        }
        p.num_tiles = best_rounds * num_cus;
    }
    p.rows_per_slot_tile = 32 + p.ex;
    return p;
}

}
```

### fullsubnet_plus_amd/csrc/lstm_common.h

```cpp
#pragma once
#include "fsnp_common.h"

namespace fsnp {

using f32x16 = __attribute__((ext_vector_type(16))) float;

__device__ __forceinline__ float fast_sigmoid(float x) { return __builtin_amdgcn_rcpf(1.0f + __expf(-x)); }
__device__ __forceinline__ float fast_tanh(float x) { return 2.0f * __builtin_amdgcn_rcpf(1.0f + __expf(-2.0f * x)) - 1.0f; }

using f32x2 = __attribute__((ext_vector_type(2))) float;
__device__ __forceinline__ f32x2 exp2_pair(f32x2 x) { return f32x2{__builtin_amdgcn_exp2f(x.x), __builtin_amdgcn_exp2f(x.y)}; }
__device__ __forceinline__ f32x2 rcp_pair(f32x2 x) { return f32x2{__builtin_amdgcn_rcpf(x.x), __builtin_amdgcn_rcpf(x.y)}; }
__device__ __forceinline__ f32x2 min_pair(f32x2 x, float m) { return f32x2{fminf(x.x, m), fminf(x.y, m)}; }
__device__ __forceinline__ f32x2 lstm_cell_pair(f32x2 xi, f32x2 xf, f32x2 xg, f32x2 xo, f32x2& c) {
    constexpr float kS = -1.4426950408889634f, kT = -2.8853900817779268f;
    const f32x2 ei = exp2_pair(xi * kS), ef = exp2_pair(xf * kS), eo = exp2_pair(xo * kS);
    const f32x2 eg = exp2_pair(min_pair(xg * kT, 64.0f));
    const f32x2 igg = (1.0f - eg) * rcp_pair((1.0f + ei) * (1.0f + eg));
    const f32x2 cn = rcp_pair(1.0f + ef) * c + igg;
    c = cn;
    const f32x2 ec = exp2_pair(min_pair(cn * kT, 64.0f));
    return (1.0f - ec) * rcp_pair((1.0f + eo) * (1.0f + ec));
}

__device__ __forceinline__ f32x2 gru_cell_pair(f32x2 ar, f32x2 az, f32x2 anx, f32x2 anh, f32x2 h) {
    constexpr float kS = -1.4426950408889634f, kT = -2.8853900817779268f;
    const f32x2 r = rcp_pair(1.0f + exp2_pair(ar * kS));
    const f32x2 ez = exp2_pair(min_pair(az * kS, 60.0f));
    const f32x2 en = exp2_pair(min_pair((anx + r * anh) * kT, 60.0f));
    const f32x2 num = ez * (1.0f - en) + h * (1.0f + en);
    return num * rcp_pair((1.0f + ez) * (1.0f + en));
}

__device__ __forceinline__ float apply_act(float v, int act) {
    if (act == FSNP_ACT_RELU) return fmaxf(v, 0.0f);
    if (act == FSNP_ACT_RELU6) return fminf(fmaxf(v, 0.0f), 6.0f);
    if (act == FSNP_ACT_TANH) return tanhf(v);
    return v;
}

__host__ __device__ __forceinline__ int a_frag_index(int row, int k) {
    return (((k >> 3) * 64) + ((k & 1) * 32) + row) * 4 + ((k >> 1) & 3);
}


constexpr int kCoopCounterStride = 64;
#define FSNP_COOP_BAR(a, tile, which) ((a).coop_bar_stride ? (a).coop_bar + (size_t)(tile) * (a).coop_bar_stride + (which) * ((a).coop_bar_stride / 2) \
                                                           : ((which) ? (a).coop_bar2 : (a).coop_bar) + (tile))
__host__ __device__ constexpr size_t coop_counter_bytes(int tiles) { return (size_t)tiles * kCoopCounterStride * 4; }
__host__ __device__ constexpr int coop_tile_f4(int HID) { return 5 * (HID / 8) * 64 + 2 * (HID / 8) * 16; }

__host__ __device__ __forceinline__ int xcd_local_tiles(int S, int T, int cus_per_xcd) {
    const int fit = cus_per_xcd / S, need = (T + 7) / 8;
    return fit < need ? fit : need;
}
__host__ __device__ __forceinline__ int xcd_local_blocks_per_xcd(int S, int T, int cus_per_xcd) {
    const int Lx = xcd_local_tiles(S, T, cus_per_xcd);
    const int t_local = T < 8 * Lx ? T : 8 * Lx;
    return Lx * S + ((T - t_local) * S + 7) / 8;
}
__device__ __forceinline__ bool xcd_local_decode(int id, int S, int T, int cus_per_xcd, int& tile, int& cs) {
    const int Lx = xcd_local_tiles(S, T, cus_per_xcd);
    const int t_local = T < 8 * Lx ? T : 8 * Lx;
    const int xcd = id & 7, j = id >> 3;
    if (j < Lx * S) { tile = (j / S) * 8 + xcd; cs = j % S; return tile < t_local; }
    const int q = (j - Lx * S) * 8 + xcd;
    tile = t_local + q / S; cs = q % S;
    return tile < T;
}

constexpr int kSc1 = 16;
__device__ __forceinline__ void xchg_store(float* p, float v) {
    __hip_atomic_store(p, v, __ATOMIC_RELAXED, __HIP_MEMORY_SCOPE_AGENT);
}
__device__ __forceinline__ float xchg_load(const float* p) {
    return __hip_atomic_load(p, __ATOMIC_RELAXED, __HIP_MEMORY_SCOPE_AGENT);
}

constexpr long long kXchgTimeoutTicks = 200000000LL;
__device__ __forceinline__ bool xchg_wait(const unsigned* bar, unsigned target, unsigned* abort_dev, unsigned* err_host) {
    unsigned spins = 0;
    long long t0 = 0;
    while (__hip_atomic_load(bar, __ATOMIC_RELAXED, __HIP_MEMORY_SCOPE_AGENT) < target) {
        __builtin_amdgcn_s_sleep(1);
        if ((++spins & 255u) == 0) {
            if (__hip_atomic_load(abort_dev, __ATOMIC_RELAXED, __HIP_MEMORY_SCOPE_AGENT) != 0) return false;
            const long long now = wall_clock64();
            if (t0 == 0) t0 = now;
            else if (now - t0 > kXchgTimeoutTicks) {
                __hip_atomic_store(abort_dev, 1u, __ATOMIC_RELAXED, __HIP_MEMORY_SCOPE_AGENT);
                __hip_atomic_store(err_host, 1u, __ATOMIC_RELAXED, __HIP_MEMORY_SCOPE_SYSTEM);
                return false;
            }
        }
    }
    return true;
}

__device__ __forceinline__ void chaos_delay(int seed, int t, int phase) {
    if (seed == 0) return;
    unsigned h = (unsigned)seed * 2654435761u ^ (unsigned)blockIdx.x * 40503u ^ (unsigned)t * 2246822519u ^ (unsigned)phase * 3266489917u;
    h ^= h >> 15; h *= 2246822519u; h ^= h >> 13; h *= 3266489917u; h ^= h >> 16;
    int n = 0;
    if ((h & 7u) == 0) n = 1 + (int)((h >> 3) & 7u);
    if ((h & 1023u) == 1u) n = 64;
    for (int i = 0; i < n; ++i) __builtin_amdgcn_s_sleep(127);
}

}
```

### fullsubnet_plus_amd/csrc/weight_layouts.h

```cpp
#pragma once
#include <cstdint>
#include <cstring>
#include <vector>

#if defined(__HIPCC__) || defined(__CUDACC__)
#define FSNP_HD __host__ __device__
#else
#define FSNP_HD
#endif

namespace fsnp {

constexpr int kFbvXP = 288;
constexpr int kFbvK0 = 100, kFbvK1 = 128;

enum PackKind : int {
    PK_ROWTILE = 0,
    PK_ROWTILE_BF,
    PK_HALF,
    PK_HALF_BF,
    PK_GRU,
    PK_KSPLIT,
    PK_COOPN,
    PK_HP,
    PK_HPW,
    PK_COOPW,
    PK_FBV,
    PK_GENERIC,
    PK_BIAS,
    PK_SPREAD,
    PK_PADMAT,
    PK_TRANSPOSE,
    PK_FOLDW,
    PK_FOLDC,
    PK_COUNT
};

struct PackJob {
    int kind;
    int p[8];
    long long s[8];
    long long out, n, sub;
    int nsub, nb;
    long long stride_in, stride_out;
};

enum PackOp : int { OP_ONE = 0, OP_ADD = 1, OP_DMUL = 2 };
struct PackRef {
    int a; long long ia;
    int b; long long ib;
    int op;
};
FSNP_HD inline PackRef ref_zero() { return PackRef{-1, 0, -1, 0, OP_ONE}; }
FSNP_HD inline PackRef ref_one(int a, long long ia) { return PackRef{a, ia, -1, 0, OP_ONE}; }

FSNP_HD inline PackRef rnn_w(const int* p, int m, long long row, long long k) {
    const int H = p[0], cols = m == 0 ? p[1] : H;
    if (p[4]) {
        const int slot = (int)(row / H);
        const bool hidden = (m & 1) != 0;
        if (slot == 2 && hidden) return ref_zero();
        if (slot == 3) { if (!hidden) return ref_zero(); row -= H; }
    }
    return ref_one(m, row * cols + k);
}
FSNP_HD inline PackRef rnn_bias(const int* p, int l, long long i) {
    const int H = p[0];
    if (!p[4] || i < 2 * H) return PackRef{4 + 2 * l, i, 5 + 2 * l, i, OP_ADD};
    if (i < 3 * H) return ref_one(4 + 2 * l, i);
    return ref_one(5 + 2 * l, i - H);
}

FSNP_HD inline int coop_kgxp(int KX) { return (KX / 8 + 3) / 4 * 4; }
FSNP_HD inline int gx16(int KX) { return (KX + 15) / 16; }

FSNP_HD inline long long pack_floats(int kind, const int* p) {
    const long long H = p[0], KX = p[2], P = p[3];
    switch (kind) {
    case PK_ROWTILE: return P * (KX / 8 + 3 * (H / 8)) * (4 * (H / P / 32)) * 256;
    case PK_ROWTILE_BF: return P * (KX / 8 + 2 * (H / 8) + H / 16) * (4 * (H / P / 32)) * 256;
    case PK_HALF: return 4 * (gx16((int)KX) + 3 * (H / 16)) * (4 * (H / 4 / 16)) * 256;
    case PK_HALF_BF: return 4 * (gx16((int)KX) + 2 * (H / 16) + H / 32) * (4 * (H / 4 / 16)) * 256;
    case PK_GRU: return P * (KX / 8 + 3 * (H / 8)) * (3 * (H / P / 32)) * 256;
    case PK_KSPLIT: return (H / P) * 4 * ((coop_kgxp((int)KX) + H / 8) / 4 + H / 16) * (P / 8) * 256;
    case PK_COOPN: return (H / 32) * (KX / 8 + 3 * (H / 8)) * 4 * 256;
    case PK_HP: case PK_HPW: return (H / 16) * 4 * (gx16((int)KX) + 3 * (H / 16)) * 256;
    case PK_COOPW: return (KX / 8 + 3 * (H / 8)) * (H / 8) * 256;
    case PK_FBV: return (H / 8) * (kFbvK0 + kFbvK1) * 256;
    case PK_GENERIC: return ((long long)p[1] + H) * 4 * H + 2 * H * 4 * H;
    case PK_BIAS: return 8 * H;
    case PK_SPREAD: return 4 * H * (p[3] == 0 ? p[1] : H);
    case PK_PADMAT: case PK_FOLDW: return (long long)p[2] * p[3];
    case PK_TRANSPOSE: return (long long)p[0] * p[1];
    case PK_FOLDC: return p[2];
    default: return 0;
    }
}

FSNP_HD inline bool pack_unit_bf16(const PackJob& J, long long u) {
    const int H = J.p[0], KX = J.p[2];
    if (J.kind == PK_ROWTILE_BF) {
        const int NW = J.p[3], NT = 4 * (H / NW / 32), KGH = H / 8, KG0 = KX / 8 + KGH, KGT = KG0 + KGH + H / 16;
        return u < J.n / 4 && (int)((u / 64 / NT) % KGT) >= KG0 + KGH;
    }
    if (J.kind == PK_HALF_BF) {
        const int NT = 4 * (H / 4 / 16), KGH = H / 16, KG0 = gx16(KX) + KGH, KGT = KG0 + KGH + H / 32;
        return u < J.n / 4 && (int)((u / 64 / NT) % KGT) >= KG0 + KGH;
    }
    return false;
}

FSNP_HD inline PackRef pack_ref(const PackJob& J, long long u, int j, long long* shift) {
    *shift = 0;
    const int* p = J.p;
    const int H = p[0], NIN = p[1], KX = p[2], P = p[3];
    const bool bf = pack_unit_bf16(J, u);
    long long pos = bf ? 4 * u : 4 * u + j;
    if (pos >= J.sub * J.nsub) return ref_zero();
    if (J.nsub > 1 || J.sub != J.n) {
        const long long bi = pos / J.sub;
        pos -= bi * J.sub;
        *shift = (bi / J.nb) * J.stride_out + (bi % J.nb) * J.stride_in;
    }
    const int c4 = (int)(pos & 3), lane = (int)((pos >> 2) & 63);
    const long long t = pos >> 8;
    switch (J.kind) {
    case PK_ROWTILE: case PK_ROWTILE_BF: case PK_COOPN: case PK_COOPW: {
        const int KGX = KX / 8, KGH = H / 8, KG0 = KGX + KGH;
        long long wrow; int g;
        if (J.kind == PK_COOPN) {
            const int KGT = KG0 + 2 * KGH, gate = (int)(t % 4);
            g = (int)((t / 4) % KGT);
            wrow = (long long)gate * H + (t / 4 / KGT) * 32 + (lane & 31);
        } else if (J.kind == PK_COOPW) {
            const int NUB = H / 8, c = lane & 31;
            g = (int)(t / NUB);
            wrow = (long long)(c & 3) * H + (t % NUB) * 8 + (c >> 2);
        } else {
            const int UW = H / P, ST = UW / 32, NT = 4 * ST;
            const int KGT = J.kind == PK_ROWTILE ? KG0 + 2 * KGH : KG0 + KGH + H / 16;
            const int n = (int)(t % NT), wv = (int)(t / NT / KGT);
            g = (int)((t / NT) % KGT);
            wrow = (long long)(n / ST) * H + wv * UW + (n % ST) * 32 + (lane & 31);
        }
        if (g < KG0) {
            const int k = 8 * g + 2 * c4 + (lane >> 5);
            if (k >= KX) return rnn_w(p, 1, wrow, k - KX);
            if (k < NIN) return rnn_w(p, 0, wrow, k);
            if (J.kind == PK_ROWTILE_BF && k == NIN) return rnn_bias(p, 0, wrow);
            return ref_zero();
        }
        if (bf) return rnn_w(p, 2, wrow, 16 * (g - KG0 - KGH) + 8 * (lane >> 5) + j);
        const int k = 8 * (g - KG0) + 2 * c4 + (lane >> 5);
        return k < H ? rnn_w(p, 3, wrow, k) : rnn_w(p, 2, wrow, k - H);
    }
    case PK_HALF: case PK_HALF_BF: {
        const int UW = H / 4, SB = UW / 16, NT = 4 * SB, KGX = gx16(KX), KGH = H / 16, KG0 = KGX + KGH;
        const int KGT = J.kind == PK_HALF ? KG0 + 2 * KGH : KG0 + KGH + H / 32;
        const int n = (int)(t % NT), g = (int)((t / NT) % KGT), wv = (int)(t / NT / KGT);
        const long long wrow = (long long)(n / SB) * H + wv * UW + (n % SB) * 16 + (lane & 15);
        if (bf) return rnn_w(p, 2, wrow, 32 * (g - KG0 - KGH) + 8 * (lane >> 4) + j);
        const int kk = 4 * c4 + (lane >> 4);
        if (g < KGX) { const int k = 16 * g + kk; return k < NIN ? rnn_w(p, 0, wrow, k) : ref_zero(); }
        if (g < KG0) return rnn_w(p, 1, wrow, 16 * (g - KGX) + kk);
        if (g < KG0 + KGH) return rnn_w(p, 3, wrow, 16 * (g - KG0) + kk);
        return rnn_w(p, 2, wrow, 16 * (g - KG0 - KGH) + kk);
    }
    case PK_GRU: {
        const int UW = H / P, ST = UW / 32, NL = 3 * ST, KGX = KX / 8, KGH = H / 8, KG0 = KGX + KGH, KGT = KG0 + 2 * KGH;
        const int n = (int)(t % NL), g = (int)((t / NL) % KGT), wv = (int)(t / NL / KGT);
        const bool l0 = g < KG0, hidden = l0 ? g >= KGX : g < KG0 + KGH;
        const int m = l0 ? (hidden ? 1 : 0) : (hidden ? 3 : 2);
        const int cols = m == 0 ? NIN : H;
        const int g0 = l0 ? (hidden ? KGX : 0) : (hidden ? KG0 : KG0 + KGH);
        const int slot = n < 2 * ST ? n / ST : (hidden ? 3 : 2);
        const long long wrow = (long long)slot * H + wv * UW + (n % ST) * 32 + (lane & 31);
        const int k = 8 * (g - g0) + 2 * c4 + (lane >> 5);
        return k < cols ? rnn_w(p, m, wrow, k) : ref_zero();
    }
    case PK_KSPLIT: {
        const int units = P, NT = units / 8, KGXP = coop_kgxp(KX), KGH = H / 8, G0W = (KGXP + KGH) / 4, GW = G0W + KGH / 2;
        const int n = (int)(t % NT), i = (int)((t / NT) % GW), wave = (int)((t / NT / GW) % 4), cs = (int)(t / NT / GW / 4);
        const int col = n * 32 + (lane & 31);
        const long long wrow = (long long)(col / units) * H + cs * units + col % units;
        if (i < G0W) {
            const int g = 4 * i + wave;
            if (g < KGXP) { const int k = 8 * g + 2 * c4 + (lane >> 5); return k < NIN ? rnn_w(p, 0, wrow, k) : ref_zero(); }
            return rnn_w(p, 1, wrow, 8 * (g - KGXP) + 2 * c4 + (lane >> 5));
        }
        const int k = 8 * (4 * (i - G0W) + wave) + 2 * c4 + (lane >> 5);
        return k < H ? rnn_w(p, 3, wrow, k) : rnn_w(p, 2, wrow, k - H);
    }
    case PK_HP: case PK_HPW: {
        const int GX = gx16(KX), GH = H / 16, NF = GX + 3 * GH;
        const int f = (int)(t % NF);
        long long wrow;
        if (J.kind == PK_HP) {
            const long long cg = t / NF;
            wrow = (cg % 4) * H + (cg / 4) * 16 + (lane & 15);
        } else {
            const long long part = t / NF;
            const int m = lane & 15;
            wrow = (long long)(m & 3) * H + (part >> 2) * 16 + (part & 3) + 4 * (m >> 2);
        }
        const int kk = 4 * c4 + (lane >> 4);
        if (f < GX) { const int k = 16 * f + kk; return k < NIN ? rnn_w(p, 0, wrow, k) : ref_zero(); }
        if (f < GX + GH) return rnn_w(p, 1, wrow, 16 * (f - GX) + kk);
        if (f < GX + 2 * GH) return rnn_w(p, 3, wrow, 16 * (f - GX - GH) + kk);
        return rnn_w(p, 2, wrow, 16 * (f - GX - 2 * GH) + kk);
    }
    case PK_FBV: {
        const int NF = (kFbvK0 + kFbvK1) / 4;
        const int tid = (int)((pos >> 2) & 255), f = (int)((pos >> 10) % NF), cs = (int)((pos >> 10) / NF);
        const int c = tid & 31, ks = tid >> 5, jj = 4 * f + c4;
        const long long wrow = (long long)(c & 3) * H + cs * 8 + (c >> 2);
        if (jj < kFbvK0) {
            const int k = kFbvK0 * ks + jj;
            if (k >= kFbvXP) return rnn_w(p, 1, wrow, k - kFbvXP);
            return k < NIN ? rnn_w(p, 0, wrow, k) : ref_zero();
        }
        const int k = kFbvK1 * ks + (jj - kFbvK0);
        return k < H ? rnn_w(p, 2, wrow, k) : rnn_w(p, 3, wrow, k - H);
    }
    case PK_GENERIC: {
        const long long G4 = 4LL * H, L0 = (NIN + (long long)H) * G4;
        if (pos < L0) { const long long k = pos / G4, c = pos % G4; return k < NIN ? rnn_w(p, 0, c, k) : rnn_w(p, 1, c, k - NIN); }
        const long long k = (pos - L0) / G4, c = (pos - L0) % G4;
        return k < H ? rnn_w(p, 2, c, k) : rnn_w(p, 3, c, k - H);
    }
    case PK_BIAS: return rnn_bias(p, (int)(pos / (4LL * H)), pos % (4LL * H));
    case PK_SPREAD: { const int cols = P == 0 ? NIN : H; return rnn_w(p, P, pos / cols, pos % cols); }
    case PK_PADMAT: case PK_FOLDW: {
        const long long n = pos / p[3], k = pos % p[3];
        if (n >= p[0] || k >= p[1]) return ref_zero();
        if (J.kind == PK_PADMAT) return ref_one(0, n * p[1] + k);
        return PackRef{0, n * p[1] + k, 1, k, OP_DMUL};
    }
    case PK_TRANSPOSE: return ref_one(0, (pos % p[0]) * p[1] + pos / p[0]);
    default: return ref_zero();
    }
}

FSNP_HD inline unsigned short bf16_rne(float v) {
    unsigned u;
#if defined(__HIP_DEVICE_COMPILE__)
    u = __float_as_uint(v);
#else
    memcpy(&u, &v, 4);
#endif
    return (unsigned short)((u + 0x7FFFu + ((u >> 16) & 1u)) >> 16);
}

FSNP_HD inline double mul_rn(double a, double b) {
#if defined(__HIP_DEVICE_COMPILE__)
    return __dmul_rn(a, b);
#else
    volatile double r = a * b;
    return r;
#endif
}
FSNP_HD inline double add_rn(double a, double b) {
#if defined(__HIP_DEVICE_COMPILE__)
    return __dadd_rn(a, b);
#else
    volatile double r = a + b;
    return r;
#endif
}

FSNP_HD inline float pack_value(const PackJob& J, const float* arena, const PackRef& r, long long shift) {
    if (r.a < 0) return 0.0f;
    const float x = arena[J.s[r.a] + shift + r.ia];
    if (r.op == OP_ONE) return x;
    const float y = arena[J.s[r.b] + shift + r.ib];
    if (r.op == OP_ADD) return x + y;
    return (float)mul_rn((double)x, (double)y);
}

FSNP_HD inline void pack_unit(const PackJob& J, const float* arena, long long u, float* dst) {
    long long shift;
    if (pack_unit_bf16(J, u)) {
        unsigned short* d16 = reinterpret_cast<unsigned short*>(dst);
        for (int j = 0; j < 8; ++j) { const PackRef r = pack_ref(J, u, j, &shift); d16[j] = bf16_rne(pack_value(J, arena, r, shift)); }
        return;
    }
    for (int j = 0; j < 4; ++j) { const PackRef r = pack_ref(J, u, j, &shift); dst[j] = pack_value(J, arena, r, shift); }
}

FSNP_HD inline float fold_row(const PackJob& J, const float* arena, long long row) {
    if (row >= J.sub * J.nsub) return 0.0f;
    const long long bi = row / J.sub, n = row % J.sub;
    const long long shift = (bi / J.nb) * J.stride_out + (bi % J.nb) * J.stride_in;
    const int R = J.p[0], C = J.p[1], which = J.p[3];
    if (n >= R) return 0.0f;
    const float* w = arena + J.s[0] + shift + n * C;
    const float* v = arena + J.s[which ? 1 : 2] + shift;
    double acc = which ? 0.0 : (double)arena[J.s[3] + shift + n];
    for (int k = 0; k < C; ++k) acc = add_rn(acc, mul_rn((double)v[k], (double)w[k]));
    return (float)acc;
}

inline PackJob make_job(int kind, int p0, int p1 = 0, int p2 = 0, int p3 = 0, int p4 = 0) {
    PackJob J{};
    J.kind = kind;
    J.p[0] = p0; J.p[1] = p1; J.p[2] = p2; J.p[3] = p3; J.p[4] = p4;
    J.sub = J.n = pack_floats(kind, J.p);
    J.nsub = 1; J.nb = 1;
    return J;
}

inline void pack_image_host(const PackJob& J, const float* arena, float* out, long long count) {
    if (J.kind == PK_FOLDC) {
        for (long long r = 0; r < count; ++r) out[r] = fold_row(J, arena, r);
        return;
    }
    for (long long u = 0; 4 * u < count; ++u) {
        if (4 * u + 4 <= count) { pack_unit(J, arena, u, out + 4 * u); continue; }
        float tmp[4];
        pack_unit(J, arena, u, tmp);
        memcpy(out + 4 * u, tmp, (size_t)(count - 4 * u) * 4);
    }
}

inline long long rnn_image_floats(int kind, int H, int NIN, int KX, int P) { return make_job(kind, H, NIN, KX, P, 0).n; }
inline void pack_rnn_host(int kind, int H, int NIN, int KX, int P, const float* wih0, const float* whh0, const float* wih1, const float* whh1,
                          float* out) {
    PackJob J = make_job(kind, H, NIN, KX, P, 0);
    const float* src[4] = {wih0, whh0, wih1, whh1};
    std::vector<float> arena;
    for (int i = 0; i < 4; ++i) {
        J.s[i] = (long long)arena.size();
        arena.insert(arena.end(), src[i], src[i] + (size_t)4 * H * (i == 0 ? NIN : H));
    }
    pack_image_host(J, arena.data(), out, J.n);
}

int launch_pack_image(const PackJob& J, const float* d_arena, long long arena_floats, float* d_blob, long long count, void* hip_stream);

}
```

### fullsubnet_plus_amd/csrc/weight_pack.hip

```cpp
#include "fsnp_common.h"
#include "weight_layouts.h"

namespace fsnp {

template <int KIND>
__global__ __launch_bounds__(256) void pack_image_kernel(PackJob J, const float* __restrict__ arena, long long arena_floats,
                                                         float* __restrict__ blob, long long units) {
    const long long u = (long long)blockIdx.x * 256 + threadIdx.x;
    if (u >= units) return;
    J.kind = KIND;
    long long shift;
    auto value = [&](int j) {
        const PackRef r = pack_ref(J, u, j, &shift);
        if (r.a < 0) return 0.0f;
        const long long ia = J.s[r.a] + shift + r.ia;
        if (ia < 0 || ia >= arena_floats) return 0.0f;
        const float x = arena[ia];
        if (r.op == OP_ONE) return x;
        const long long ib = J.s[r.b] + shift + r.ib;
        if (ib < 0 || ib >= arena_floats) return 0.0f;
        const float y = arena[ib];
        return r.op == OP_ADD ? x + y : (float)mul_rn((double)x, (double)y);
    };
    uint4 o;
    if ((KIND == PK_ROWTILE_BF || KIND == PK_HALF_BF) && pack_unit_bf16(J, u)) {
        unsigned w[4];
        for (int q = 0; q < 4; ++q) w[q] = (unsigned)bf16_rne(value(2 * q)) | ((unsigned)bf16_rne(value(2 * q + 1)) << 16);
        o = make_uint4(w[0], w[1], w[2], w[3]);
    } else {
        o = make_uint4(__float_as_uint(value(0)), __float_as_uint(value(1)), __float_as_uint(value(2)), __float_as_uint(value(3)));
    }
    reinterpret_cast<uint4*>(blob + J.out)[u] = o;
}

__global__ __launch_bounds__(64) void pack_fold_kernel(PackJob J, const float* __restrict__ arena, float* __restrict__ blob, long long rows) {
    const long long r = (long long)blockIdx.x * 64 + threadIdx.x;
    if (r < rows) blob[J.out + r] = fold_row(J, arena, r);
}

template <int KIND>
static void launch_kind(const PackJob& J, const float* arena, long long arena_floats, float* blob, long long units, hipStream_t s) {
    hipLaunchKernelGGL(pack_image_kernel<KIND>, dim3((unsigned)((units + 255) / 256)), dim3(256), 0, s, J, arena, arena_floats, blob, units);
}

int launch_pack_image(const PackJob& J, const float* d_arena, long long arena_floats, float* d_blob, long long count, void* hip_stream) {
    hipStream_t s = static_cast<hipStream_t>(hip_stream);
    if (count <= 0) return 0;
    if (count % 4 != 0 || J.out % 4 != 0) { set_error("weight pack: image of kind %d is not a whole number of 16-byte units", J.kind); return 3; }
    if (J.kind == PK_FOLDC) {
        const long long last = (long long)(J.nsub - 1) / J.nb * J.stride_out + (long long)(J.nsub - 1) % J.nb * J.stride_in;
        if (J.nsub > 0 && (J.s[0] + last + (long long)J.p[0] * J.p[1] > arena_floats || J.s[1] + last + J.p[1] > arena_floats ||
                           J.s[2] + last + J.p[1] > arena_floats || J.s[3] + last + J.p[0] > arena_floats)) {
            set_error("weight pack: a GroupNorm fold reads outside the arena"); return 3;
        }
        hipLaunchKernelGGL(pack_fold_kernel, dim3((unsigned)((count + 63) / 64)), dim3(64), 0, s, J, d_arena, d_blob, count);
        FSNP_HIP_CHECK(hipGetLastError());
        return 0;
    }
    const long long units = count / 4;
    switch (J.kind) {
    case PK_ROWTILE: launch_kind<PK_ROWTILE>(J, d_arena, arena_floats, d_blob, units, s); break;
    case PK_ROWTILE_BF: launch_kind<PK_ROWTILE_BF>(J, d_arena, arena_floats, d_blob, units, s); break;
    case PK_HALF: launch_kind<PK_HALF>(J, d_arena, arena_floats, d_blob, units, s); break;
    case PK_HALF_BF: launch_kind<PK_HALF_BF>(J, d_arena, arena_floats, d_blob, units, s); break;
    case PK_GRU: launch_kind<PK_GRU>(J, d_arena, arena_floats, d_blob, units, s); break;
    case PK_KSPLIT: launch_kind<PK_KSPLIT>(J, d_arena, arena_floats, d_blob, units, s); break;
    case PK_COOPN: launch_kind<PK_COOPN>(J, d_arena, arena_floats, d_blob, units, s); break;
    case PK_HP: launch_kind<PK_HP>(J, d_arena, arena_floats, d_blob, units, s); break;
    case PK_HPW: launch_kind<PK_HPW>(J, d_arena, arena_floats, d_blob, units, s); break;
    case PK_COOPW: launch_kind<PK_COOPW>(J, d_arena, arena_floats, d_blob, units, s); break;
    case PK_FBV: launch_kind<PK_FBV>(J, d_arena, arena_floats, d_blob, units, s); break;
    case PK_GENERIC: launch_kind<PK_GENERIC>(J, d_arena, arena_floats, d_blob, units, s); break;
    case PK_BIAS: launch_kind<PK_BIAS>(J, d_arena, arena_floats, d_blob, units, s); break;
    case PK_SPREAD: launch_kind<PK_SPREAD>(J, d_arena, arena_floats, d_blob, units, s); break;
    case PK_PADMAT: launch_kind<PK_PADMAT>(J, d_arena, arena_floats, d_blob, units, s); break;
    case PK_TRANSPOSE: launch_kind<PK_TRANSPOSE>(J, d_arena, arena_floats, d_blob, units, s); break;
    case PK_FOLDW: launch_kind<PK_FOLDW>(J, d_arena, arena_floats, d_blob, units, s); break;
    default: set_error("weight pack: unknown image kind %d", J.kind); return 3;
    }
    FSNP_HIP_CHECK(hipGetLastError());
    return 0;
}

}
```

Before: 146,800.

## Pre-scale LSTM gate weights by -log2e factors and fold bias into input column

Adds scaled row-tile weight pack kinds that multiply gate weights by -log2(e) (or -2log2(e) for the cell gate) at pack time. The cell nonlinearities then use exp2 directly without a per-element multiply. Layer-0 bias moves into a constant-1 input column, and the first MFMA group starts from a zero accumulator instead of bias-initialised registers. This removes per-step VALU work for scaling and bias setup in the recurrent kernel, at the cost of more template variants and changes to weight-pack semantics.

Result: no change. 147,900 (median of 6 runs) (+0.7%).

```diff
diff --git a/fullsubnet_plus_amd/csrc/fsnp_debug_abi.hip b/fullsubnet_plus_amd/csrc/fsnp_debug_abi.hip
--- a/fullsubnet_plus_amd/csrc/fsnp_debug_abi.hip
+++ b/fullsubnet_plus_amd/csrc/fsnp_debug_abi.hip
@@ -445,13 +445,14 @@
         if (sizes[i] < 0) { set_error("fsnp_debug_pack_emulate: negative size"); return 2; }
         p[i] = sizes[i];
     }
-    const bool rnn = kind <= PK_SPREAD;
+    const bool rnn = kind <= PK_SPREAD || kind == PK_ROWTILE_S || kind == PK_ROWTILE_BF_S;
     const int want_sources = rnn ? 8 : kind == PK_FOLDW ? 2 : kind == PK_FOLDC ? 4 : 1;
     bool ok = p[0] > 0 && num_sources == want_sources;
     if (rnn && kind != PK_BIAS) ok = ok && p[1] > 0;
     if (kind <= PK_FBV) ok = ok && p[0] % 8 == 0;
-    if (kind == PK_ROWTILE || kind == PK_ROWTILE_BF || kind == PK_GRU) ok = ok && p[3] > 0 && p[0] % (32 * p[3]) == 0 && p[2] % 8 == 0 && p[1] <= p[2];
-    if (kind == PK_ROWTILE_BF) ok = ok && p[1] < p[2] && p[0] % 16 == 0;
+    if (kind == PK_ROWTILE_S || kind == PK_ROWTILE_BF_S) ok = ok && p[0] % 8 == 0 && p[4] == 0;
+    if (kind == PK_ROWTILE || kind == PK_ROWTILE_BF || kind == PK_GRU || kind == PK_ROWTILE_S || kind == PK_ROWTILE_BF_S) ok = ok && p[3] > 0 && p[0] % (32 * p[3]) == 0 && p[2] % 8 == 0 && p[1] <= p[2];
+    if (kind == PK_ROWTILE_BF || kind == PK_ROWTILE_BF_S) ok = ok && p[1] < p[2] && p[0] % 16 == 0;
     if (kind == PK_HALF || kind == PK_HALF_BF) ok = ok && p[0] % 64 == 0 && p[1] <= p[2];
     if (kind == PK_KSPLIT) ok = ok && p[3] >= 8 && p[3] % 8 == 0 && p[0] % p[3] == 0 && p[0] % 16 == 0 && (4 * p[3]) % 32 == 0 && p[2] % 8 == 0 && p[1] <= p[2] && (coop_kgxp(p[2]) + p[0] / 8) % 4 == 0;
     if (kind == PK_COOPN || kind == PK_COOPW) ok = ok && p[0] % 32 == 0 && p[2] % 8 == 0 && p[1] <= p[2];
diff --git a/fullsubnet_plus_amd/csrc/fsnp_weights.hip b/fullsubnet_plus_amd/csrc/fsnp_weights.hip
--- a/fullsubnet_plus_amd/csrc/fsnp_weights.hip
+++ b/fullsubnet_plus_amd/csrc/fsnp_weights.hip
@@ -346,9 +346,9 @@
     if (h->generic_sb) o_wgen = sb(PK_GENERIC);
     size_t o_wpack = 0, o_wpack12 = 0, o_wpack_bf[2] = {0, 0};
     if (!h->gru && tuned && (H == 384 || H == 256)) {
-        o_wpack = sb(PK_ROWTILE, 4);
-        if (H == 384) o_wpack12 = sb(PK_ROWTILE, 12);
-        for (int i = 0; i < 2 && h->KX == 40 && H == 384 && h->NIN < h->KX; ++i) o_wpack_bf[i] = sb(PK_ROWTILE_BF, i == 0 ? 4 : 12);
+        o_wpack = sb(PK_ROWTILE_S, 4);
+        if (H == 384) o_wpack12 = sb(PK_ROWTILE_S, 12);
+        for (int i = 0; i < 2 && h->KX == 40 && H == 384 && h->NIN < h->KX; ++i) o_wpack_bf[i] = sb(PK_ROWTILE_BF_S, i == 0 ? 4 : 12);
     }
     size_t o_wpack16 = 0, o_wpack16_bf = 0;
     bool have16_bf = false;
diff --git a/fullsubnet_plus_amd/csrc/lstm.hip b/fullsubnet_plus_amd/csrc/lstm.hip
--- a/fullsubnet_plus_amd/csrc/lstm.hip
+++ b/fullsubnet_plus_amd/csrc/lstm.hip
@@ -1,4 +1,5 @@
 #include <cstring>
+#include <type_traits>
 
 #include "fsnp_common.h"
 #include "lstm_common.h"
@@ -20,63 +21,106 @@
     return __builtin_bit_cast(float4, v);
 }
 
-template <int NT, int EX>
+template <bool ZERO>
+__device__ __forceinline__ void mfma_tile(f32x16& acc, const float4& a, const float4& b) {
+    if constexpr (ZERO) {
+        constexpr f32x16 zero = {0.f, 0.f, 0.f, 0.f, 0.f, 0.f, 0.f, 0.f, 0.f, 0.f, 0.f, 0.f, 0.f, 0.f, 0.f, 0.f};
+        acc = __builtin_amdgcn_mfma_f32_32x32x2f32(a.x, b.x, zero, 0, 0, 0);
+    } else {
+        acc = __builtin_amdgcn_mfma_f32_32x32x2f32(a.x, b.x, acc, 0, 0, 0);
+    }
+    acc = __builtin_amdgcn_mfma_f32_32x32x2f32(a.y, b.y, acc, 0, 0, 0);
+    acc = __builtin_amdgcn_mfma_f32_32x32x2f32(a.z, b.z, acc, 0, 0, 0);
+    acc = __builtin_amdgcn_mfma_f32_32x32x2f32(a.w, b.w, acc, 0, 0, 0);
+}
+
+template <int NT, int EX, bool ZERO>
+__device__ __forceinline__ void mfma_group(f32x16 (&acc)[NT], float (&accx)[EX > 0 ? EX : 1][NT], float4 (&b)[NT], const float4& a,
+                                           const float4 (&ae)[EX > 0 ? EX : 1], const WStream& ws, int gnext) {
+    if constexpr (EX == 0) {
+#pragma unroll
+        for (int n = 0; n < NT; ++n) {
+            mfma_tile<ZERO>(acc[n], a, b[n]);
+            b[n] = wload<NT>(ws, gnext, n);
+            __builtin_amdgcn_sched_barrier(0);
+        }
+    } else {
+        constexpr int HALF = NT / 2;
+#pragma unroll
+        for (int hb = 0; hb < NT; hb += HALF) {
+#pragma unroll
+            for (int n = hb; n < hb + HALF; ++n) mfma_tile<ZERO>(acc[n], a, b[n]);
+            __builtin_amdgcn_sched_barrier(0);
+#pragma unroll
+            for (int n = hb; n < hb + HALF; ++n)
+#pragma unroll
+                for (int e = 0; e < EX; ++e) {
+                    float v = accx[e][n];
+                    v = fmaf(ae[e].x, b[n].x, v);
+                    v = fmaf(ae[e].y, b[n].y, v);
+                    v = fmaf(ae[e].z, b[n].z, v);
+                    accx[e][n] = fmaf(ae[e].w, b[n].w, v);
+                }
+            __builtin_amdgcn_sched_barrier(0);
+#pragma unroll
+            for (int n = hb; n < hb + HALF; ++n) b[n] = wload<NT>(ws, gnext, n);
+            __builtin_amdgcn_sched_barrier(0);
+        }
+    }
+}
+
+template <int NT, int EX, bool START>
 __device__ __forceinline__ void mfma_groups(f32x16 (&acc)[NT], float (&accx)[EX > 0 ? EX : 1][NT], float4 (&b)[NT],
                                             const float4* __restrict__ A, const float4* __restrict__ AE, int ngroups,
                                             const WStream& ws, int& gnext, int groups_total) {
+    if constexpr (EX == 0) {
+        using f32x4 = __attribute__((ext_vector_type(4))) float;
+        const f32x4* __restrict__ Av = reinterpret_cast<const f32x4*>(A);
+        float4 ae[1] = {};
+        auto group = [&](const f32x4& v, auto zero) {
+            const float4 a = make_float4(v.x, v.y, v.z, v.w);
+            mfma_group<NT, 0, decltype(zero)::value>(acc, accx, b, a, ae, ws, gnext);
+            gnext = (gnext + 1 == groups_total) ? 0 : gnext + 1;
+        };
+        f32x4 a0 = Av[0], a1 = Av[64];
+        int g = 0;
+        if constexpr (START) {
+            group(a0, std::true_type{});
+            a0 = Av[2 * 64];
+            group(a1, std::false_type{});
+            a1 = Av[3 * 64];
+            g = 2;
+        }
+        for (; g + 3 < ngroups; g += 2) {
+            group(a0, std::false_type{});
+            a0 = Av[(g + 2) * 64];
+            group(a1, std::false_type{});
+            a1 = Av[(g + 3) * 64];
+        }
+        group(a0, std::false_type{});
+        if (g + 2 < ngroups) a0 = Av[(g + 2) * 64];
+        group(a1, std::false_type{});
+        if (g + 2 < ngroups) group(a0, std::false_type{});
+        return;
+    }
     float4 a = A[0];
     float4 ae[EX > 0 ? EX : 1];
 #pragma unroll
     for (int e = 0; e < EX; ++e) ae[e] = AE[e];
-    for (int g = 0; g < ngroups; ++g) {
+    auto step = [&](int g, auto zero) {
         const int gn = (g + 1 < ngroups ? g + 1 : g);
         const float4 an = A[gn * 64];
         float4 aen[EX > 0 ? EX : 1];
 #pragma unroll
         for (int e = 0; e < EX; ++e) aen[e] = AE[gn * 2 * EX + e];
-        if constexpr (EX == 0) {
-#pragma unroll
-            for (int n = 0; n < NT; ++n) {
-                acc[n] = __builtin_amdgcn_mfma_f32_32x32x2f32(a.x, b[n].x, acc[n], 0, 0, 0);
-                acc[n] = __builtin_amdgcn_mfma_f32_32x32x2f32(a.y, b[n].y, acc[n], 0, 0, 0);
-                acc[n] = __builtin_amdgcn_mfma_f32_32x32x2f32(a.z, b[n].z, acc[n], 0, 0, 0);
-                acc[n] = __builtin_amdgcn_mfma_f32_32x32x2f32(a.w, b[n].w, acc[n], 0, 0, 0);
-                b[n] = wload<NT>(ws, gnext, n);
-                __builtin_amdgcn_sched_barrier(0);
-            }
-        } else {
-            constexpr int HALF = NT / 2;
-#pragma unroll
-            for (int hb = 0; hb < NT; hb += HALF) {
-#pragma unroll
-                for (int n = hb; n < hb + HALF; ++n) {
-                    acc[n] = __builtin_amdgcn_mfma_f32_32x32x2f32(a.x, b[n].x, acc[n], 0, 0, 0);
-                    acc[n] = __builtin_amdgcn_mfma_f32_32x32x2f32(a.y, b[n].y, acc[n], 0, 0, 0);
-                    acc[n] = __builtin_amdgcn_mfma_f32_32x32x2f32(a.z, b[n].z, acc[n], 0, 0, 0);
-                    acc[n] = __builtin_amdgcn_mfma_f32_32x32x2f32(a.w, b[n].w, acc[n], 0, 0, 0);
-                }
-                __builtin_amdgcn_sched_barrier(0);
-#pragma unroll
-                for (int n = hb; n < hb + HALF; ++n)
-#pragma unroll
-                    for (int e = 0; e < EX; ++e) {
-                        float v = accx[e][n];
-                        v = fmaf(ae[e].x, b[n].x, v);
-                        v = fmaf(ae[e].y, b[n].y, v);
-                        v = fmaf(ae[e].z, b[n].z, v);
-                        accx[e][n] = fmaf(ae[e].w, b[n].w, v);
-                    }
-                __builtin_amdgcn_sched_barrier(0);
-#pragma unroll
-                for (int n = hb; n < hb + HALF; ++n) b[n] = wload<NT>(ws, gnext, n);
-                __builtin_amdgcn_sched_barrier(0);
-            }
-        }
+        mfma_group<NT, EX, decltype(zero)::value>(acc, accx, b, a, ae, ws, gnext);
         gnext = (gnext + 1 == groups_total) ? 0 : gnext + 1;
         a = an;
 #pragma unroll
         for (int e = 0; e < EX; ++e) ae[e] = aen[e];
-    }
+    };
+    if constexpr (START) step(0, std::true_type{});
+    for (int g = START ? 1 : 0; g < ngroups; ++g) step(g, std::false_type{});
 }
 
 __device__ __forceinline__ unsigned short bf16_bits(float v) {
@@ -87,22 +131,31 @@
     return (((k >> 4) * 64) + (((k >> 3) & 1) * 32) + row) * 8 + (k & 7);
 }
 
-template <int ST, int UW, int HBLO = 0>
-__device__ __forceinline__ void lstm_cell(f32x16 (&acc)[4 * ST], f32x2 (&c)[ST][8], float* __restrict__ Hs, int wave,
-                                          int lane, unsigned short* __restrict__ Hb = nullptr) {
+template <int ST, int UW, bool BIAS, int HBLO = 0>
+__device__ __forceinline__ void lstm_cell(f32x16 (&acc)[4 * ST], f32x2 (&c)[ST][8], const float* __restrict__ bias, float* __restrict__ Hs,
+                                          int wave, int lane, unsigned short* __restrict__ Hb = nullptr) {
 #pragma unroll
     for (int s = 0; s < ST; ++s) {
         const int k = wave * UW + s * 32 + (lane & 31);
         const int kbase = (((k >> 3) * 64) + ((k & 1) * 32)) * 4 + ((k >> 1) & 3);
+        float bq[4] = {0.0f, 0.0f, 0.0f, 0.0f};
+        if constexpr (BIAS) {
+#pragma unroll
+            for (int q = 0; q < 4; ++q) bq[q] = bias[(q * ST + s) * 32];
+        }
 #pragma unroll
         for (int r = 0; r < 16; r += 2) {
             auto rd = [](float v) {
                 if constexpr (ST > 1) { float o; asm("v_accvgpr_read_b32 %0, %1" : "=v"(o) : "a"(v)); return o; }
                 else return v;
             };
-            const f32x2 h = lstm_cell_pair(f32x2{rd(acc[s][r]), rd(acc[s][r + 1])}, f32x2{rd(acc[ST + s][r]), rd(acc[ST + s][r + 1])},
-                                           f32x2{rd(acc[2 * ST + s][r]), rd(acc[2 * ST + s][r + 1])},
-                                           f32x2{rd(acc[3 * ST + s][r]), rd(acc[3 * ST + s][r + 1])}, c[s][r >> 1]);
+            f32x2 g4[4];
+#pragma unroll
+            for (int q = 0; q < 4; ++q) {
+                g4[q] = f32x2{rd(acc[q * ST + s][r]), rd(acc[q * ST + s][r + 1])};
+                if constexpr (BIAS) g4[q] += bq[q];
+            }
+            const f32x2 h = lstm_cell_pair_scaled(g4[0], g4[1], g4[2], g4[3], c[s][r >> 1]);
             const int row = (r & 3) + 8 * (r >> 2) + 4 * (lane >> 5);
             Hs[kbase + row * 4] = h.x;
             Hs[kbase + (row + 1) * 4] = h.y;
@@ -177,17 +230,18 @@
                 const float v = accx[e][q * ST + s];
                 g4[q] = v + __shfl_xor(v, 32) + (bias ? bias[(q * ST + s) * 32] : 0.0f);
             }
-            const float cn = fast_sigmoid(g4[1]) * cx[e][s] + fast_sigmoid(g4[0]) * fast_tanh(g4[2]);
+            const float cn = sigmoid_scaled(g4[1]) * cx[e][s] + sigmoid_scaled(g4[0]) * tanh_scaled(g4[2]);
             cx[e][s] = cn;
-            const float h = fast_sigmoid(g4[3]) * fast_tanh(cn);
+            const float h = sigmoid_scaled(g4[3]) * fast_tanh(cn);
             if (lane < 32) He[e_frag_index<EX>(e, wave * UW + s * 32 + lane)] = h;
         }
 }
 
-template <int HID, int KX, int OUT, int EX, bool PROF, int NW, bool BF>
+template <int HID, int KX, int OUT, int EX, bool PROF, int NW, bool BF, bool BCOL>
 __global__ __launch_bounds__(64 * NW) __attribute__((amdgpu_waves_per_eu(NW / 4, NW / 4)))
 void lstm2_fc_kernel(LstmWeights w, LstmArgs a) {
     static_assert(OUT == 2, "FC lane mapping assumes output_size == 2");
+    static_assert(BCOL || !BF, "the bf16-ih variant has no bias table for layer 0");
     static_assert(EX >= 0 && EX <= 4, "at most 4 VALU rows per tile (one FC wave per extra row)");
     static_assert(NW % 4 == 0 && NW >= 4, "whole waves per SIMD");
     constexpr int NTHR = 64 * NW;
@@ -210,6 +264,7 @@
     float4* HE1s = HE0s + KGH * 2 * EX;
     float4* Wfc4 = HE1s + KGH * 2 * EX;
     RowDesc* rows_s = reinterpret_cast<RowDesc*>(Wfc4 + OUT * KGH * 2);
+    constexpr bool bcol = BCOL;
     constexpr int BL = BF ? 1 : 2;
     constexpr bool HILO = BF && EX == 0;
     float* Bs = reinterpret_cast<float*>(rows_s + RT);
@@ -237,10 +292,10 @@
     if (tid < RT) rows_s[tid] = a.rows[slot0 + tid];
     for (int i = tid; i < BL * NW * NT * 32; i += NTHR) {
         const int col = i & 31, n = (i >> 5) % NT, wv = (i / (32 * NT)) % NW, layer = BF ? 1 : i / (32 * NT * NW);
-        Bs[i] = w.bias[layer * 4 * HID + (n / ST) * HID + wv * UW + (n % ST) * 32 + col];
+        Bs[i] = w.bias[layer * 4 * HID + (n / ST) * HID + wv * UW + (n % ST) * 32 + col] * (n / ST == 2 ? kGateScaleT : kGateScaleS);
     }
     __syncthreads();
-    if constexpr (BF) {
+    if (bcol) {
         if (tid < 32) reinterpret_cast<float*>(Xs)[a_frag_index(tid, w.NIN)] = 1.0f;
         if (EX > 0 && tid < EX) reinterpret_cast<float*>(XEs)[e_frag_index<EXA>(tid, w.NIN)] = 1.0f;
     }
@@ -268,7 +323,7 @@
 #pragma unroll
         for (int i = 0; i < NG; ++i) {
             const int j = (tid >> 5) + JSTEP * i;
-            goff[i] = (j < KX && !(BF && j == w.NIN)) ? plan(rd, j) : -2;
+            goff[i] = (j < KX && !(bcol && j == w.NIN)) ? plan(rd, j) : -2;
             xdst[i] = a_frag_index(grow, j < KX ? j : 0);
         }
         row_md(rd, slot0 + grow, md, md_row);
@@ -276,7 +331,7 @@
     int goffx = -1, xdstx = 0;
     NormMD mdx = {0.0f, 1.0f}; const NormMD* mdx_row = nullptr;
     bool havex = EX > 0 && tid < EX * KX;
-    if (BF && havex && tid % KX == w.NIN) havex = false;
+    if (bcol && havex && tid % KX == w.NIN) havex = false;
     if (havex) {
         const int e = tid / KX, j = tid % KX;
         const RowDesc rd = rows_s[32 + e];
@@ -298,7 +353,7 @@
         }
     }
 
-    const float* __restrict__ bias_l0 = BF ? nullptr : Bs + ((0 * NW + wave) * NT) * 32 + (lane & 31);
+    const float* __restrict__ bias_l0 = bcol ? nullptr : Bs + ((0 * NW + wave) * NT) * 32 + (lane & 31);
     const float* __restrict__ bias_l1 = Bs + (((BL - 1) * NW + wave) * NT) * 32 + (lane & 31);
     f32x2 c0[ST][8], c1[ST][8];
     float cx0[EXA][ST], cx1[EXA][ST];
@@ -318,8 +373,8 @@
 #pragma unroll
     for (int n = 0; n < NT; ++n) breg[n] = wload<NT>(ws, 0, n);
     int gnext = 1;
-    auto run_groups = [&](f32x16 (&acc_)[NT], float (&accx_)[EXA][NT], const float4* A_, const float4* AE_, int ng) {
-        mfma_groups<NT, EX>(acc_, accx_, breg, A_, AE_, ng, ws, gnext, KGT);
+    auto run_groups = [&](f32x16 (&acc_)[NT], float (&accx_)[EXA][NT], const float4* A_, const float4* AE_, int ng, auto start) {
+        mfma_groups<NT, EX, decltype(start)::value>(acc_, accx_, breg, A_, AE_, ng, ws, gnext, KGT);
     };
 
     const int fc_row = (wave & 3) * 8 + (lane & 7);
@@ -396,17 +451,15 @@
         f32x16 acc[NT];
         float accx[EXA][NT];
 #pragma unroll
-        for (int n = 0; n < NT; ++n) {
-#pragma unroll
-            for (int r = 0; r < 16; ++r) acc[n][r] = BF ? 0.0f : bias_l0[n * 32];
+        for (int n = 0; n < NT; ++n)
 #pragma unroll
             for (int e = 0; e < EXA; ++e) accx[e][n] = 0.0f;
-        }
-        run_groups(acc, accx, Xs + lane, AEx, KG0);
+        run_groups(acc, accx, Xs + lane, AEx, KG0, std::true_type{});
         FSNP_STAMP(1);
         __syncthreads();
         FSNP_STAMP(2);
-        lstm_cell<ST, UW, HILO ? KSB * 64 * 8 : 0>(acc, c0, reinterpret_cast<float*>(H0s), wave, lane, BF ? reinterpret_cast<unsigned short*>(H0b) : nullptr);
+        lstm_cell<ST, UW, !BCOL, HILO ? KSB * 64 * 8 : 0>(acc, c0, bias_l0, reinterpret_cast<float*>(H0s), wave, lane,
+                                                          BF ? reinterpret_cast<unsigned short*>(H0b) : nullptr);
         if (EX > 0) lstm_cell_extra<ST, UW, EX, NT>(accx, cx0, bias_l0, reinterpret_cast<float*>(HE0s), wave, lane);
         if (have_next) {
 #pragma unroll
@@ -419,19 +472,16 @@
         __syncthreads();
         FSNP_STAMP(4);
 #pragma unroll
-        for (int n = 0; n < NT; ++n) {
-#pragma unroll
-            for (int r = 0; r < 16; ++r) acc[n][r] = bias_l1[n * 32];
+        for (int n = 0; n < NT; ++n)
 #pragma unroll
             for (int e = 0; e < EXA; ++e) accx[e][n] = 0.0f;
-        }
-        run_groups(acc, accx, H1s + lane, AEh1, KGH);
+        run_groups(acc, accx, H1s + lane, AEh1, KGH, std::true_type{});
         if constexpr (BF) mfma_groups_bf16<NT, EX, HILO ? KSB * 64 : 0>(acc, accx, breg, H0b + lane, HE0s, KSB, ws, gnext, KGT, lane);
-        else run_groups(acc, accx, H0s + lane, AEh0, KGH);
+        else run_groups(acc, accx, H0s + lane, AEh0, KGH, std::false_type{});
         FSNP_STAMP(5);
         __syncthreads();
         FSNP_STAMP(6);
-        lstm_cell<ST, UW>(acc, c1, reinterpret_cast<float*>(H1s), wave, lane);
+        lstm_cell<ST, UW, true>(acc, c1, bias_l1, reinterpret_cast<float*>(H1s), wave, lane);
         if (EX > 0) lstm_cell_extra<ST, UW, EX, NT>(accx, cx1, bias_l1, reinterpret_cast<float*>(HE1s), wave, lane);
         FSNP_STAMP(7);
     }
@@ -451,23 +501,26 @@
 
 
 
-template <int EX, int NW, bool BF, int KX, int HID = 384>
+template <int EX, int NW, bool BF, int KX, int HID = 384, bool BCOL = true>
 static void launch_lstm_ex(const LstmWeights& w, const LstmArgs& a, hipStream_t s) {
     constexpr int OUT = 2;
     constexpr int KGX = KX / 8, KGH = HID / 8, NT = 4 * (HID / NW / 32);
     const size_t smem = (size_t)(KGX + 2 * KGH) * (64 + 2 * EX) * 16 + (size_t)OUT * KGH * 2 * 16 +
                         (32 + EX) * sizeof(RowDesc) + (size_t)(BF ? 1 : 2) * NW * NT * 32 * 4 + (BF ? (size_t)(EX == 0 ? 2 : 1) * (HID / 16) * 64 * 16 : 0);
+    if constexpr (!BF && BCOL) {
+        if (w.NIN >= KX) { launch_lstm_ex<EX, NW, BF, KX, HID, false>(w, a, s); return; }
+    }
     LstmWeights wv = w;
     wv.wpack = BF ? (NW == 12 ? w.wpack_bf[1] : w.wpack_bf[0]) : (NW == 12 ? w.wpack12 : w.wpack);
     if constexpr (KX == 40 && HID == 384) {
         if (a.prof != nullptr) {
-            auto kern = lstm2_fc_kernel<HID, KX, OUT, EX, true, NW, BF>;
+            auto kern = lstm2_fc_kernel<HID, KX, OUT, EX, true, NW, BF, BCOL>;
             (void)hipFuncSetAttribute(reinterpret_cast<const void*>(kern), hipFuncAttributeMaxDynamicSharedMemorySize, (int)smem);
             hipLaunchKernelGGL(kern, dim3(a.num_tiles), dim3(64 * NW), smem, s, wv, a);
             return;
         }
     }
-    auto kern = lstm2_fc_kernel<HID, KX, OUT, EX, false, NW, BF>;
+    auto kern = lstm2_fc_kernel<HID, KX, OUT, EX, false, NW, BF, BCOL>;
     static PerDeviceOnce attr_once;
     attr_once.run([&] { (void)hipFuncSetAttribute(reinterpret_cast<const void*>(kern), hipFuncAttributeMaxDynamicSharedMemorySize, (int)smem); });
     hipLaunchKernelGGL(kern, dim3(a.num_tiles), dim3(64 * NW), smem, s, wv, a);
@@ -532,7 +585,7 @@
     }
 }
 
-template <int HID, int KX>
+template <int HID, int KX, bool BCOL>
 __global__ __launch_bounds__(256) __attribute__((amdgpu_waves_per_eu(1, 1)))
 void lstm2_fc_stream_kernel(LstmWeights w, LstmArgs a) {
     constexpr int NW = 4, NTHR = 256, OUT = 2;
@@ -563,9 +616,11 @@
     if (tid < 32) rows_s[tid] = a.rows[slot0 + tid];
     for (int i = tid; i < 2 * NW * NT * 32; i += NTHR) {
         const int col = i & 31, n = (i >> 5) % NT, wv = (i / (32 * NT)) % NW, layer = i / (32 * NT * NW);
-        Bs[i] = w.bias[layer * 4 * HID + (n / ST) * HID + wv * UW + (n % ST) * 32 + col];
+        Bs[i] = w.bias[layer * 4 * HID + (n / ST) * HID + wv * UW + (n % ST) * 32 + col] * (n / ST == 2 ? kGateScaleT : kGateScaleS);
     }
     __syncthreads();
+    constexpr bool bcol = BCOL;
+    if (bcol && tid < 32) reinterpret_cast<float*>(Xs)[a_frag_index(tid, w.NIN)] = 1.0f;
 
     int nsteps = 0, cmin = 1 << 30;
     for (int r = 0; r < 32; ++r) {
@@ -588,7 +643,7 @@
 #pragma unroll
         for (int i = 0; i < NG; ++i) {
             const int j = (tid >> 5) + JSTEP * i;
-            goff[i] = j >= KX ? -2 : (rd.valid > 0 && j < w.NIN)
+            goff[i] = (j >= KX || (bcol && j == w.NIN)) ? -2 : (rd.valid > 0 && j < w.NIN)
                           ? sb_feature_offset(j, rd.f, rd.b * Tp * a.FP, a.F, a.NSBN, a.NFBN, a.fb_rel, a.fb_branch_stride) : -1;
             xdst[i] = a_frag_index(grow, j < KX ? j : 0);
         }
@@ -616,8 +671,8 @@
     for (int n = 0; n < NT; ++n) breg[n] = wload<NT>(ws, 0, n);
     int gnext = 1;
     float accx[1][NT];
-    auto run_groups = [&](f32x16 (&acc_)[NT], const float4* A_, int ng) {
-        mfma_groups<NT, 0>(acc_, accx, breg, A_, A_, ng, ws, gnext, KGT);
+    auto run_groups = [&](f32x16 (&acc_)[NT], const float4* A_, int ng, auto start) {
+        mfma_groups<NT, 0, decltype(start)::value>(acc_, accx, breg, A_, A_, ng, ws, gnext, KGT);
     };
 
     const int fc_row = (wave & 3) * 8 + (lane & 7);
@@ -656,13 +711,9 @@
         }
 
         f32x16 acc[NT];
-#pragma unroll
-        for (int n = 0; n < NT; ++n)
-#pragma unroll
-            for (int r = 0; r < 16; ++r) acc[n][r] = bias_l0[n * 32];
-        run_groups(acc, Xs + lane, KG0);
+        run_groups(acc, Xs + lane, KG0, std::true_type{});
         __syncthreads();
-        lstm_cell<ST, UW>(acc, c0, reinterpret_cast<float*>(H0s), wave, lane);
+        lstm_cell<ST, UW, !BCOL>(acc, c0, bias_l0, reinterpret_cast<float*>(H0s), wave, lane);
         if (have_next) {
 #pragma unroll
             for (int i = 0; i < NG; ++i)
@@ -670,14 +721,10 @@
         }
         if (t > 0) fc_store(t - 1);
         __syncthreads();
-#pragma unroll
-        for (int n = 0; n < NT; ++n)
-#pragma unroll
-            for (int r = 0; r < 16; ++r) acc[n][r] = bias_l1[n * 32];
-        run_groups(acc, H1s + lane, KGH);
-        run_groups(acc, H0s + lane, KGH);
+        run_groups(acc, H1s + lane, KGH, std::true_type{});
+        run_groups(acc, H0s + lane, KGH, std::false_type{});
         __syncthreads();
-        lstm_cell<ST, UW>(acc, c1, reinterpret_cast<float*>(H1s), wave, lane);
+        lstm_cell<ST, UW, true>(acc, c1, bias_l1, reinterpret_cast<float*>(H1s), wave, lane);
         if (t + 1 == nsteps || mixed)
             stream_state_io<ST, UW, HID, false>(c0, c1, reinterpret_cast<float*>(H0s), reinterpret_cast<float*>(H1s), rows_s, a.st_sb,
                                                 a.st_stride, t + 1, wave, lane);
@@ -686,11 +733,14 @@
     fc_store(nsteps - 1);
 }
 
-template <int HID, int KX>
+template <int HID, int KX, bool BCOL = true>
 static void launch_lstm_stream_one(const LstmWeights& w, const LstmArgs& a, hipStream_t s) {
+    if constexpr (BCOL) {
+        if (w.NIN >= KX) { launch_lstm_stream_one<HID, KX, false>(w, a, s); return; }
+    }
     constexpr int KGX = KX / 8, KGH = HID / 8, NT = 4 * (HID / 4 / 32);
     const size_t smem = (size_t)(KGX + 2 * KGH) * 64 * 16 + (size_t)2 * KGH * 2 * 16 + 32 * sizeof(RowDesc) + (size_t)2 * 4 * NT * 32 * 4;
-    auto kern = lstm2_fc_stream_kernel<HID, KX>;
+    auto kern = lstm2_fc_stream_kernel<HID, KX, BCOL>;
     static PerDeviceOnce attr_once;
     attr_once.run([&] { (void)hipFuncSetAttribute(reinterpret_cast<const void*>(kern), hipFuncAttributeMaxDynamicSharedMemorySize, (int)smem); });
     hipLaunchKernelGGL(kern, dim3(a.num_tiles), dim3(256), smem, s, w, a);
diff --git a/fullsubnet_plus_amd/csrc/lstm_common.h b/fullsubnet_plus_amd/csrc/lstm_common.h
--- a/fullsubnet_plus_amd/csrc/lstm_common.h
+++ b/fullsubnet_plus_amd/csrc/lstm_common.h
@@ -1,5 +1,6 @@
 #pragma once
 #include "fsnp_common.h"
+#include "weight_layouts.h"
 
 namespace fsnp {
 
@@ -22,6 +23,18 @@
     const f32x2 ec = exp2_pair(min_pair(cn * kT, 64.0f));
     return (1.0f - ec) * rcp_pair((1.0f + eo) * (1.0f + ec));
 }
+
+__device__ __forceinline__ f32x2 lstm_cell_pair_scaled(f32x2 si, f32x2 sf, f32x2 sg, f32x2 so, f32x2& c) {
+    const f32x2 ei = exp2_pair(si), ef = exp2_pair(sf), eo = exp2_pair(so);
+    const f32x2 eg = min_pair(exp2_pair(sg), 0x1p64f);
+    const f32x2 igg = (1.0f - eg) * rcp_pair((1.0f + ei) * (1.0f + eg));
+    const f32x2 cn = rcp_pair(1.0f + ef) * c + igg;
+    c = cn;
+    const f32x2 ec = exp2_pair(min_pair(cn * kGateScaleT, 64.0f));
+    return (1.0f - ec) * rcp_pair((1.0f + eo) * (1.0f + ec));
+}
+__device__ __forceinline__ float sigmoid_scaled(float s) { return __builtin_amdgcn_rcpf(1.0f + __builtin_amdgcn_exp2f(s)); }
+__device__ __forceinline__ float tanh_scaled(float s) { return 2.0f * __builtin_amdgcn_rcpf(1.0f + __builtin_amdgcn_exp2f(s)) - 1.0f; }
 
 __device__ __forceinline__ f32x2 gru_cell_pair(f32x2 ar, f32x2 az, f32x2 anx, f32x2 anh, f32x2 h) {
     constexpr float kS = -1.4426950408889634f, kT = -2.8853900817779268f;
diff --git a/fullsubnet_plus_amd/csrc/weight_layouts.h b/fullsubnet_plus_amd/csrc/weight_layouts.h
--- a/fullsubnet_plus_amd/csrc/weight_layouts.h
+++ b/fullsubnet_plus_amd/csrc/weight_layouts.h
@@ -33,8 +33,12 @@
     PK_TRANSPOSE,
     PK_FOLDW,
     PK_FOLDC,
+    PK_ROWTILE_S,
+    PK_ROWTILE_BF_S,
     PK_COUNT
 };
+
+constexpr float kGateScaleS = -1.4426950408889634f, kGateScaleT = -2.8853900817779268f;
 
 struct PackJob {
     int kind;
@@ -77,8 +81,8 @@
 FSNP_HD inline long long pack_floats(int kind, const int* p) {
     const long long H = p[0], KX = p[2], P = p[3];
     switch (kind) {
-    case PK_ROWTILE: return P * (KX / 8 + 3 * (H / 8)) * (4 * (H / P / 32)) * 256;
-    case PK_ROWTILE_BF: return P * (KX / 8 + 2 * (H / 8) + H / 16) * (4 * (H / P / 32)) * 256;
+    case PK_ROWTILE: case PK_ROWTILE_S: return P * (KX / 8 + 3 * (H / 8)) * (4 * (H / P / 32)) * 256;
+    case PK_ROWTILE_BF: case PK_ROWTILE_BF_S: return P * (KX / 8 + 2 * (H / 8) + H / 16) * (4 * (H / P / 32)) * 256;
     case PK_HALF: return 4 * (gx16((int)KX) + 3 * (H / 16)) * (4 * (H / 4 / 16)) * 256;
     case PK_HALF_BF: return 4 * (gx16((int)KX) + 2 * (H / 16) + H / 32) * (4 * (H / 4 / 16)) * 256;
     case PK_GRU: return P * (KX / 8 + 3 * (H / 8)) * (3 * (H / P / 32)) * 256;
@@ -99,7 +103,7 @@
 
 FSNP_HD inline bool pack_unit_bf16(const PackJob& J, long long u) {
     const int H = J.p[0], KX = J.p[2];
-    if (J.kind == PK_ROWTILE_BF) {
+    if (J.kind == PK_ROWTILE_BF || J.kind == PK_ROWTILE_BF_S) {
         const int NW = J.p[3], NT = 4 * (H / NW / 32), KGH = H / 8, KG0 = KX / 8 + KGH, KGT = KG0 + KGH + H / 16;
         return u < J.n / 4 && (int)((u / 64 / NT) % KGT) >= KG0 + KGH;
     }
@@ -125,7 +129,7 @@
     const int c4 = (int)(pos & 3), lane = (int)((pos >> 2) & 63);
     const long long t = pos >> 8;
     switch (J.kind) {
-    case PK_ROWTILE: case PK_ROWTILE_BF: case PK_COOPN: case PK_COOPW: {
+    case PK_ROWTILE: case PK_ROWTILE_BF: case PK_ROWTILE_S: case PK_ROWTILE_BF_S: case PK_COOPN: case PK_COOPW: {
         const int KGX = KX / 8, KGH = H / 8, KG0 = KGX + KGH;
         long long wrow; int g;
         if (J.kind == PK_COOPN) {
@@ -138,7 +142,7 @@
             wrow = (long long)(c & 3) * H + (t % NUB) * 8 + (c >> 2);
         } else {
             const int UW = H / P, ST = UW / 32, NT = 4 * ST;
-            const int KGT = J.kind == PK_ROWTILE ? KG0 + 2 * KGH : KG0 + KGH + H / 16;
+            const int KGT = (J.kind == PK_ROWTILE || J.kind == PK_ROWTILE_S) ? KG0 + 2 * KGH : KG0 + KGH + H / 16;
             const int n = (int)(t % NT), wv = (int)(t / NT / KGT);
             g = (int)((t / NT) % KGT);
             wrow = (long long)(n / ST) * H + wv * UW + (n % ST) * 32 + (lane & 31);
@@ -147,7 +151,7 @@
             const int k = 8 * g + 2 * c4 + (lane >> 5);
             if (k >= KX) return rnn_w(p, 1, wrow, k - KX);
             if (k < NIN) return rnn_w(p, 0, wrow, k);
-            if (J.kind == PK_ROWTILE_BF && k == NIN) return rnn_bias(p, 0, wrow);
+            if ((J.kind == PK_ROWTILE_BF || J.kind == PK_ROWTILE_S || J.kind == PK_ROWTILE_BF_S) && k == NIN) return rnn_bias(p, 0, wrow);
             return ref_zero();
         }
         if (bf) return rnn_w(p, 2, wrow, 16 * (g - KG0 - KGH) + 8 * (lane >> 5) + j);
@@ -241,6 +245,13 @@
     }
 }
 
+FSNP_HD inline float pack_scale(const PackJob& J, long long u) {
+    if (J.kind != PK_ROWTILE_S && J.kind != PK_ROWTILE_BF_S) return 1.0f;
+    const int ST = J.p[0] / J.p[3] / 32;
+    return (int)((u / 64) % (4 * ST)) / ST == 2 ? kGateScaleT : kGateScaleS;
+}
+FSNP_HD inline float pack_scaled(float v, float scale) { return scale == 1.0f ? v : v * scale; }
+
 FSNP_HD inline unsigned short bf16_rne(float v) {
     unsigned u;
 #if defined(__HIP_DEVICE_COMPILE__)
@@ -279,12 +290,13 @@
 
 FSNP_HD inline void pack_unit(const PackJob& J, const float* arena, long long u, float* dst) {
     long long shift;
+    const float sc = pack_scale(J, u);
     if (pack_unit_bf16(J, u)) {
         unsigned short* d16 = reinterpret_cast<unsigned short*>(dst);
-        for (int j = 0; j < 8; ++j) { const PackRef r = pack_ref(J, u, j, &shift); d16[j] = bf16_rne(pack_value(J, arena, r, shift)); }
+        for (int j = 0; j < 8; ++j) { const PackRef r = pack_ref(J, u, j, &shift); d16[j] = bf16_rne(pack_scaled(pack_value(J, arena, r, shift), sc)); }
         return;
     }
-    for (int j = 0; j < 4; ++j) { const PackRef r = pack_ref(J, u, j, &shift); dst[j] = pack_value(J, arena, r, shift); }
+    for (int j = 0; j < 4; ++j) { const PackRef r = pack_ref(J, u, j, &shift); dst[j] = pack_scaled(pack_value(J, arena, r, shift), sc); }
 }
 
 FSNP_HD inline float fold_row(const PackJob& J, const float* arena, long long row) {
diff --git a/fullsubnet_plus_amd/csrc/weight_pack.hip b/fullsubnet_plus_amd/csrc/weight_pack.hip
--- a/fullsubnet_plus_amd/csrc/weight_pack.hip
+++ b/fullsubnet_plus_amd/csrc/weight_pack.hip
@@ -10,7 +10,8 @@
     if (u >= units) return;
     J.kind = KIND;
     long long shift;
-    auto value = [&](int j) {
+    const float sc = pack_scale(J, u);
+    auto raw = [&](int j) {
         const PackRef r = pack_ref(J, u, j, &shift);
         if (r.a < 0) return 0.0f;
         const long long ia = J.s[r.a] + shift + r.ia;
@@ -22,8 +23,9 @@
         const float y = arena[ib];
         return r.op == OP_ADD ? x + y : (float)mul_rn((double)x, (double)y);
     };
+    auto value = [&](int j) { return pack_scaled(raw(j), sc); };
     uint4 o;
-    if ((KIND == PK_ROWTILE_BF || KIND == PK_HALF_BF) && pack_unit_bf16(J, u)) {
+    if ((KIND == PK_ROWTILE_BF || KIND == PK_ROWTILE_BF_S || KIND == PK_HALF_BF) && pack_unit_bf16(J, u)) {
         unsigned w[4];
         for (int q = 0; q < 4; ++q) w[q] = (unsigned)bf16_rne(value(2 * q)) | ((unsigned)bf16_rne(value(2 * q + 1)) << 16);
         o = make_uint4(w[0], w[1], w[2], w[3]);
@@ -76,6 +78,8 @@
     case PK_PADMAT: launch_kind<PK_PADMAT>(J, d_arena, arena_floats, d_blob, units, s); break;
     case PK_TRANSPOSE: launch_kind<PK_TRANSPOSE>(J, d_arena, arena_floats, d_blob, units, s); break;
     case PK_FOLDW: launch_kind<PK_FOLDW>(J, d_arena, arena_floats, d_blob, units, s); break;
+    case PK_ROWTILE_S: launch_kind<PK_ROWTILE_S>(J, d_arena, arena_floats, d_blob, units, s); break;
+    case PK_ROWTILE_BF_S: launch_kind<PK_ROWTILE_BF_S>(J, d_arena, arena_floats, d_blob, units, s); break;
     default: set_error("weight pack: unknown image kind %d", J.kind); return 3;
     }
     FSNP_HIP_CHECK(hipGetLastError());
```
